# JGI-Bioinformatics/Kmernator

Measured on AMD Instinct MI355X. Metric: total k-mers/sec at k=31, 150 bp reads (spectrum build, inputs resident in HBM), higher is better.
Workload: dtype u64

## Files before the change

kmernator_amd/csrc/kmr_api.hip:

```cpp
#include <hip/hip_runtime.h>
#include <dlfcn.h>
#include <unistd.h>
#include <rccl/rccl.h>

#include <algorithm>
#include <atomic>
#include <cmath>
#include <cstdio>
#include <cstdlib>
#include <cstring>
#include <cctype>
#include <memory>
#include <mutex>
#include <string>
#include <type_traits>
#include <vector>

#include "kmr_host.hpp"
#include "kmr_kernels.hpp"
#include "kmr_partition.hpp"
#include "kmr_superkmer.hpp"
#include "kmr_buckets.hpp"
#include "kmr_synth.hpp"
#define KMR_INSTANCES_EXTERN
// ... 29 lines not shown
		if (i < 33 + (int)minQ) P[raw] = 0.0;
		else if (i < 103) P[raw] = 1.0 - pow(10.0, ((33 - i) / 10.0));
		else P[raw] = 1.0;
	}
}

}

namespace {

template <int W, class F> auto with_win(uint32_t win, F &&f) {
	if (W > 1 && win == 32) return f(int_c<(W > 1 ? 32 : 16)>());
	return win == 16 ? f(int_c<16>()) : (win == 8 ? f(int_c<8>()) : f(int_c<4>()));
}

size_t slot_bytes(kmr_handle *h) { return with_w(h, [](auto W) { return sizeof(Slot<W()>); }); }

ReadsView reads_view(const void *bases, const void *quals, const void *offsets, uint64_t n_reads, const void *discarded = nullptr, uint64_t stream_base = 0, uint64_t first_read_idx = 0) {
	ReadsView rv{};
	rv.bases = (const uint8_t *)bases; rv.quals = (const uint8_t *)quals; rv.offsets = (const uint64_t *)offsets; rv.discarded = (const uint8_t *)discarded;
	rv.n_reads = n_reads; rv.stream_base = stream_base; rv.first_read_idx = first_read_idx;
	return rv;
}
ReadsView reads_slice(const ReadsView &all, uint64_t r, uint64_t m) {
	ReadsView rv = all;
	rv.offsets = all.offsets + r; rv.n_reads = m; rv.discarded = all.discarded ? all.discarded + r : nullptr; rv.first_read_idx = all.first_read_idx + r;
	return rv;
}
FinalizeParams finalize_params(kmr_handle *h, uint32_t min_depth) {
	FinalizeParams f{};
	f.kb = h->hkb; f.ext_min_q = h->cfg.ext_min_quality; f.min_depth = min_depth; f.has_singletons = h->cfg.separate_singletons ? 1 : 0; f.nb_weak = h->nb_weak; f.nb_sing = h->nb_sing;
	return f;
}

DevParams dev_params(kmr_handle *h) {
	DevParams p;
	p.k = h->k; p.kb = h->hkb; p.min_weight = h->cfg.min_weight; p.fastq_start = h->cfg.fastq_start_char; p.ext_min_q = h->cfg.ext_min_quality;
	p.qzero = h->cfg.fastq_start_char + std::max<uint32_t>(1u, h->cfg.min_quality_score);
	p.subsample = h->cfg.kmer_subsample; p.rank = h->cfg.rank; p.world = h->cfg.world_size; p.num_parts = h->cfg.num_parts; p.part_idx = h->cfg.part_idx;
	p.count_sender_bad = h->sender_launch ? 1u : 0u;
	p.P = h->dP.get<double>(); p.stats = h->dstats.get<DevStats>(); p.err = h->derr.get<uint32_t>();
	p.sub_wstart = p.sub_wkeys = p.sub_sstart = p.sub_skeys = nullptr; p.sub_wvals = nullptr; p.sub_sweight = nullptr; p.sub_wnb = p.sub_snb = 0; p.sub_vw = 0;
	if (h->subtract) {
		const kmr_handle *o = h->subtract;
		if (o->weak.present && o->weak.n) { p.sub_wstart = o->weak.start.get<uint64_t>(); p.sub_wkeys = o->weak.keys.get<uint64_t>(); p.sub_wvals = o->weak.vals.get<uint32_t>(); p.sub_wnb = o->weak.nb; p.sub_vw = o->ext ? 15 : 3; }
		if (o->sing.present && o->sing.n) { p.sub_sstart = o->sing.start.get<uint64_t>(); p.sub_skeys = o->sing.keys.get<uint64_t>(); p.sub_sweight = o->sing.sweight.get<uint8_t>(); p.sub_snb = o->sing.nb; }
	}
	return p;
}


template <int W> Table<W> table_of(kmr_handle *h) { Table<W> t; t.slots = h->slots.get<Slot<W>>(); t.ext = h->extslots.get<ExtSlot>(); t.log2cap = h->log2cap; return t; }

template <int W> int clear_table(kmr_handle *h, void *slots, ExtSlot *ext, uint32_t log2cap) {
	hipLaunchKernelGGL(table_clear_kernel<W>, dim3(grid_for(1ull << log2cap)), dim3(256), 0, h->stream, (Slot<W> *)slots, ext, 1ull << log2cap);
	HIPCHK(h, hipGetLastError());
	return 0;
}
int clear_table_any(kmr_handle *h, void *slots, ExtSlot *ext, uint32_t log2cap) { return with_w(h, [&](auto W) { return clear_table<W()>(h, slots, ext, log2cap); }); }

int alloc_table(kmr_handle *h, uint32_t log2cap, DevBuf &slots, DevBuf &ext) {
	DevBuf s, x;
	HIPCHK(h, s.alloc(slot_bytes(h) << log2cap));
	if (h->ext) HIPCHK(h, x.alloc(sizeof(ExtSlot) << log2cap));
	const int rc = clear_table_any(h, s.get(), x.get<ExtSlot>(), log2cap);
	if (rc) return rc;
	slots = std::move(s); ext = std::move(x);
	return 0;
}

int sync_state(kmr_handle *h) {
	HIPCHK(h, hipStreamSynchronize(h->stream));
	for (int which = 0; which < KMR_TIME_GROUPS; which++) {
		for (auto &pr : h->pending_events[which]) {
			float ms = 0; hipEventElapsedTime(&ms, pr.first, pr.second);
			h->ms[which] += ms; h->launches[which]++;
			hipEventDestroy(pr.first); hipEventDestroy(pr.second);
		}
		h->pending_events[which].clear();
	}
	uint32_t e = 0; DevStats s;
	HIPCHK(h, hipMemcpy(&e, h->derr.get<uint32_t>(), sizeof(e), hipMemcpyDeviceToHost));
	HIPCHK(h, hipMemcpy(&s, h->dstats.get<DevStats>(), sizeof(s), hipMemcpyDeviceToHost));
#ifdef KMR_DEBUG_HOOKS
	if (h->superkmer_mode) { if (dbg()) fprintf(stderr, "sk_extract windows: %llu general, %llu fast\n", s.claimed, s.inserted); s.claimed = 0; s.inserted = 0; }
#endif
	h->stats.raw_kmers = s.raw + s.inserted + s.sender_bad; h->stats.raw_good_kmers = s.good + s.inserted; h->stats.discarded = s.raw - s.good + s.sender_bad;
	h->occupied = s.claimed; h->pending_kmers = 0; h->subtracted = s.subtracted;
	if (e & ERR_READ_TOO_LONG) return fail(h, KMR_ERR_UNSUPPORTED, "a read is longer than the per-wavefront LDS tile (" + std::to_string(TILE_SPAN) + " bases)");
	if (e & ERR_TABLE_FULL) return fail(h, KMR_ERR_CAPACITY, "device k-mer table is full; raise kmr_config.max_table_entries / estimated_raw_kmers");
	if (e & ERR_SEGMENT_OVERFLOW) return fail(h, KMR_ERR_CAPACITY, "an owner segment overflowed seg_capacity");
	if (e & ERR_POOL_FULL) return fail(h, KMR_ERR_CAPACITY, "record pool overflow (internal sizing error)");
	if (e & ERR_ENTRIES_FULL) return fail(h, KMR_ERR_CAPACITY, "entry buffer overflow (internal sizing error)");
	return 0;
}

template <int W, bool EXT> int grow_table_t(kmr_handle *h, uint32_t newlog) {
	DevBuf ns, ne;
	int rc = alloc_table(h, newlog, ns, ne);
	if (rc) return rc;
	Table<W> src = table_of<W>(h), dst; dst.slots = ns.get<Slot<W>>(); dst.ext = ne.get<ExtSlot>(); dst.log2cap = newlog;
	hipLaunchKernelGGL((rehash_kernel<W, EXT>), dim3(grid_for(1ull << h->log2cap)), dim3(256), 0, h->stream, src, dst, h->hkb, h->derr.get<uint32_t>());
	HIPCHK(h, hipGetLastError());
	HIPCHK(h, hipStreamSynchronize(h->stream));
	h->slots = std::move(ns); h->extslots = std::move(ne); h->log2cap = newlog;
	return 0;
}
int grow_table(kmr_handle *h, uint32_t newlog) { return with_w_ext(h, [&](auto W, auto EXT) { return grow_table_t<W(), EXT()>(h, newlog); }); }

int ensure_capacity(kmr_handle *h, uint64_t incoming) {
	const uint64_t cap = 1ull << h->log2cap;
	if ((double)(h->occupied + h->pending_kmers + incoming) <= 0.85 * (double)cap) { h->pending_kmers += incoming; return 0; }
	int rc = sync_state(h);
	if (rc) return rc;
	if ((double)(h->occupied + incoming) > 0.85 * (double)cap) {
		uint32_t nl = h->log2cap;
		while ((double)(h->occupied + incoming) > 0.6 * (double)(1ull << nl)) nl++;
		rc = grow_table(h, nl);
		if (rc) return rc;
	}
	h->pending_kmers = incoming;
	return 0;
}

const size_t EXTRACT_SMEM = (size_t)WAVES_PER_BLOCK * 2 * TILE_BUF;

int prepare_units(kmr_handle *h, ReadsView &rv, uint32_t span = (uint32_t)TILE_SPAN) {
	rv.u_start = rv.u_end = rv.u_read = nullptr; rv.n_units = 0;
	const uint64_t n = rv.n_reads;
	if (n == 0) return 0;
	int rc = h->umax.reserve(h, "umax", 4); if (rc) return rc;
	HIPCHK(h, hipMemsetAsync(h->umax.get<unsigned int>(), 0, 4, h->stream));
	rc = h->ucnt.reserve(h, "ucnt", 4 * (n + 1)); if (rc) return rc;
	hipLaunchKernelGGL(unit_count_kernel, dim3(grid_for(n)), dim3(256), 0, h->stream, rv.offsets, n, h->k, span, h->ucnt.get<uint32_t>(), h->umax.get<unsigned int>());
	HIPCHK(h, hipGetLastError());
	unsigned int mx = 0;
	HIPCHK(h, hipMemcpyAsync(&mx, h->umax.get<unsigned int>(), 4, hipMemcpyDeviceToHost, h->stream));
	HIPCHK(h, hipStreamSynchronize(h->stream));
	if (mx <= span) return 0;
	rc = h->ufirst.reserve(h, "ufirst", 8 * (n + 1)); if (rc) return rc;
	rc = exclusive_scan(h, h->ucnt.get<uint32_t>(), n, h->ufirst.get<uint64_t>()); if (rc) return rc;
	uint64_t U = 0;
	HIPCHK(h, hipMemcpy(&U, h->ufirst.get<uint64_t>() + n, 8, hipMemcpyDeviceToHost));
	if (h->u_read.cap() < 8 * U) {
		h->u_start.reset(); h->u_end.reset(); h->u_read.reset();
		HIPCHK(h, h->u_start.alloc(8 * U)); HIPCHK(h, h->u_end.alloc(8 * U)); HIPCHK(h, h->u_read.alloc(8 * U));
	}
	hipLaunchKernelGGL(unit_fill_kernel, dim3(grid_for(n)), dim3(256), 0, h->stream, rv.offsets, n, h->k, span, h->ufirst.get<uint64_t>(), h->u_start.get<uint64_t>(), h->u_end.get<uint64_t>(), h->u_read.get<uint64_t>());
	HIPCHK(h, hipGetLastError());
	rv.u_start = h->u_start.get<uint64_t>(); rv.u_end = h->u_end.get<uint64_t>(); rv.u_read = h->u_read.get<uint64_t>(); rv.n_units = U;
	return 0;
}

template <int W, bool EXT, class Op> int launch_extract(kmr_handle *h, const ReadsView &rv, const Op &op, uint64_t max_blocks = 0) {
	const DevParams dp = dev_params(h);
	const bool sub = Op::NEEDS_WEIGHT && (dp.sub_wnb | dp.sub_snb) != 0;
	auto kern = sub ? extract_kernel<W, EXT, Op, true> : extract_kernel<W, EXT, Op, false>;
	HIPCHK(h, hipFuncSetAttribute((const void *)kern, hipFuncAttributeMaxDynamicSharedMemorySize, (int)EXTRACT_SMEM));
	if (dbg()) { int nb = 0; hipOccupancyMaxActiveBlocksPerMultiprocessor(&nb, (const void *)kern, WAVES_PER_BLOCK * 64, EXTRACT_SMEM); fprintf(stderr, "extract: %d blocks of %d waves per CU (dynamic LDS %zu)\n", nb, WAVES_PER_BLOCK, EXTRACT_SMEM);
		for (size_t tr : {(size_t)79872, (size_t)65536, (size_t)52000, (size_t)38000}) { hipOccupancyMaxActiveBlocksPerMultiprocessor(&nb, (const void *)kern, WAVES_PER_BLOCK * 64, tr); fprintf(stderr, "   with %zu bytes: %d blocks\n", tr, nb); } }
	const uint64_t tiles = ((rv.u_start ? rv.n_units : rv.n_reads) + 63) / 64;
	uint64_t blocks = (tiles + WAVES_PER_BLOCK - 1) / WAVES_PER_BLOCK;
	if (blocks == 0) return 0;
	if (max_blocks && blocks > max_blocks) blocks = max_blocks;
	if (blocks > 0x7fffffffull) return fail(h, KMR_ERR_INVALID_ARG, "too many reads in one batch");
	hipLaunchKernelGGL(kern, dim3((unsigned)blocks), dim3(WAVES_PER_BLOCK * 64), EXTRACT_SMEM, h->stream, rv, dp, op);
	HIPCHK(h, hipGetLastError());
	return 0;
}

template <int W, bool EXT> int add_reads_dev_t(kmr_handle *h, const ReadsView &rvAll, uint64_t total_bases) {
	const uint64_t n = rvAll.n_reads;
	const uint64_t avg = n ? std::max<uint64_t>(1, total_bases / n) : 1;
	uint64_t chunk = std::max<uint64_t>(64, ((1ull << 27) / avg) & ~63ull);
	std::vector<uint64_t> off2(2);
	for (uint64_t r = 0; r < n; r += chunk) {
		const uint64_t m = std::min(chunk, n - r);
		HIPCHK(h, hipMemcpyAsync(&off2[0], rvAll.offsets + r, 8, hipMemcpyDeviceToHost, h->stream));
		HIPCHK(h, hipMemcpyAsync(&off2[1], rvAll.offsets + r + m, 8, hipMemcpyDeviceToHost, h->stream));
		HIPCHK(h, hipStreamSynchronize(h->stream));
		const uint64_t bases = off2[1] - off2[0];
		int rc = ensure_capacity(h, bases);
		if (rc) return rc;
		ReadsView rv = reads_slice(rvAll, r, m);
		rc = prepare_units(h, rv); if (rc) return rc;
		InsertOp<W, EXT> op; op.table = table_of<W>(h);
		TimeSpan t(h, 0);
		rc = launch_extract<W, EXT>(h, rv, op);
		t.end();
		if (rc) return rc;
	}
	return 0;
}

int add_reads_dev_any(kmr_handle *h, const ReadsView &rv, uint64_t total_bases) { return with_w_ext(h, [&](auto W, auto EXT) { return add_reads_dev_t<W(), EXT()>(h, rv, total_bases); }); }

}
namespace kmr_host {
int exclusive_scan_queue(kmr_handle *h, const uint32_t *in, uint64_t n, uint64_t *out ) {
	const uint64_t nblocks = (n + SCAN_ITEMS - 1) / SCAN_ITEMS;
	const size_t eb = sizeof(unsigned long long);
	int rc = h->scan_sums.reserve(h, "scan_sums", eb * (nblocks + 1), eb * std::max<uint64_t>(nblocks + 1, 4096)); if (rc) return rc;
	unsigned long long *sums = h->scan_sums.get<unsigned long long>(), *total = sums + nblocks;
	hipLaunchKernelGGL(scan_block_sums_kernel, dim3((unsigned)nblocks), dim3(256), 0, h->stream, in, n, sums);
	hipLaunchKernelGGL(scan_sums_kernel, dim3(1), dim3(256), 0, h->stream, sums, nblocks, total);
	hipLaunchKernelGGL(scan_apply_kernel, dim3((unsigned)nblocks), dim3(256), 0, h->stream, in, n, sums, out);
	HIPCHK(h, hipGetLastError());
	return 0;
}
int exclusive_scan(kmr_handle *h, const uint32_t *in, uint64_t n, uint64_t *out ) {
	const int rc = exclusive_scan_queue(h, in, n, out); if (rc) return rc;
	HIPCHK(h, hipStreamSynchronize(h->stream));
	return 0;
}
}
namespace {

int arena_alloc(kmr_handle *h, void **out, size_t bytes) {
	const size_t need = (bytes + 255) & ~(size_t)255;
	if (h->arena && h->arena_used + need <= h->arena.cap()) { *out = h->arena.get<uint8_t>() + h->arena_used; h->arena_used += need; h->arena_want += need; return 0; }
	h->arena_want += need;
	DevBuf b;
// ... 374 lines not shown
	const int mb = max_part_bits(h);
	int T = 0; while (T < 2 * mb && (est >> T) > TARGET_LIST_RECORDS) T++;
	h->bits1 = std::max(0, std::min(mb, T + 2 - mb));
}

template <int W, bool EXT> int extract_by_owner_t(kmr_handle *h, const ReadsView &rvAll, uint64_t total_bases, void *dev_records, uint64_t seg_capacity, void *dev_seg_counts, uint32_t *dev_pos = nullptr) {
	const uint64_t n = rvAll.n_reads;
	const uint64_t avg = n ? std::max<uint64_t>(1, total_bases / n) : 1;
	const uint64_t chunk = std::max<uint64_t>(64, (SUB_BATCH_BASES / avg) & ~63ull);
	for (uint64_t r = 0; r < n; r += chunk) {
		const uint64_t m = std::min(chunk, n - r);
		ReadsView rv = reads_slice(rvAll, r, m);
		int rc = prepare_units(h, rv); if (rc) return rc;
		const uint64_t nu = rv.u_start ? rv.n_units : m;
		rc = h->kcap.reserve(h, "kcap", 4 * std::max<uint64_t>(nu + 1, 16)); if (rc) return rc;
		rc = h->koff.reserve(h, "koff", 8 * std::max<uint64_t>(nu + 1, 16)); if (rc) return rc;
		hipLaunchKernelGGL(kmer_capacity_kernel, dim3(grid_for(nu)), dim3(256), 0, h->stream, rv, h->k, h->kcap.get<uint32_t>());
		HIPCHK(h, hipGetLastError());
		rc = exclusive_scan(h, h->kcap.get<uint32_t>(), nu, h->koff.get<uint64_t>()); if (rc) return rc;
		uint64_t total_cap = 0;
		HIPCHK(h, hipMemcpy(&total_cap, h->koff.get<uint64_t>() + nu, 8, hipMemcpyDeviceToHost));
		const uint64_t tiles = (nu + 63) / 64;
		rc = h->linear.reserve(h, "linear", sizeof(typename PoolRec<W, EXT>::type) * std::max<uint64_t>(total_cap, 16)); if (rc) return rc;
		rc = h->tile_count.reserve(h, "tile_count", 4 * std::max<uint64_t>(tiles, 16)); if (rc) return rc;
		LinearOp<W, EXT, false> op; op.records = (typename PoolRec<W, EXT>::type *)h->linear.get(); op.koff = h->koff.get<uint64_t>(); op.tile_count = h->tile_count.get<uint32_t>(); op.first_read_idx = rv.first_read_idx;
		h->sender_launch = dev_pos == nullptr;
		rc = launch_extract<W, EXT>(h, rv, op);
		h->sender_launch = false;
		if (rc) return rc;
		rc = zero_work_counter(h); if (rc) return rc;
		const int grid = (int)std::min<uint64_t>((uint64_t)num_cus(h) * 8, tiles);
		OwnerFn of; of.m = 0; of.off = of.win = of.list_bits = 0;
		if (h->superkmer_mode && h->sk_exchange) { of.m = h->sk_m; of.off = h->sk_off; of.win = h->sk_win; of.list_bits = h->sk_bits; }
		if (dev_pos)
			hipLaunchKernelGGL((owner_scatter_kernel<W, EXT, true>), dim3(grid), dim3(OWNER_THREADS), 0, h->stream, (const typename PoolRec<W, EXT>::type *)h->linear.get(), h->koff.get<uint64_t>(), h->tile_count.get<uint32_t>(), tiles, h->hkb,
			                   h->cfg.world_size, (uint32_t *)dev_records, seg_capacity, (unsigned long long *)dev_seg_counts, h->work_counter.get<unsigned int>(), h->derr.get<uint32_t>(), dev_pos, of);
		else
			hipLaunchKernelGGL((owner_scatter_kernel<W, EXT>), dim3(grid), dim3(OWNER_THREADS), 0, h->stream, (const typename PoolRec<W, EXT>::type *)h->linear.get(), h->koff.get<uint64_t>(), h->tile_count.get<uint32_t>(), tiles, h->hkb,
			                   h->cfg.world_size, (uint32_t *)dev_records, seg_capacity, (unsigned long long *)dev_seg_counts, h->work_counter.get<unsigned int>(), h->derr.get<uint32_t>(), (uint32_t *)nullptr, of);
		HIPCHK(h, hipGetLastError());
	}
	return 0;
}

template <int W, bool EXT> int add_reads_partition_t(kmr_handle *h, const ReadsView &rvAll, uint64_t total_bases) {
	const uint64_t n = rvAll.n_reads;
	if (!h->l1.head) choose_bits1(h, total_bases);
	const uint64_t avg = n ? std::max<uint64_t>(1, total_bases / n) : 1;
	const uint64_t sub_bases = h->tune.sub_batch_bases ? h->tune.sub_batch_bases : SUB_BATCH_BASES;
	const uint64_t chunk = std::max<uint64_t>(64, (sub_bases / avg) & ~63ull);
	for (uint64_t r = 0; r < n; r += chunk) {
		const uint64_t m = std::min(chunk, n - r);
		ReadsView rv = reads_slice(rvAll, r, m);
		int rc = prepare_units(h, rv); if (rc) return rc;
		const uint64_t nu = rv.u_start ? rv.n_units : m;
		rc = h->kcap.reserve(h, "kcap", 4 * std::max<uint64_t>(nu + 1, 16)); if (rc) return rc;
		rc = h->koff.reserve(h, "koff", 8 * std::max<uint64_t>(nu + 1, 16)); if (rc) return rc;
		hipLaunchKernelGGL(kmer_capacity_kernel, dim3(grid_for(nu)), dim3(256), 0, h->stream, rv, h->k, h->kcap.get<uint32_t>());
		HIPCHK(h, hipGetLastError());
		rc = exclusive_scan(h, h->kcap.get<uint32_t>(), nu, h->koff.get<uint64_t>()); if (rc) return rc;
		uint64_t total_cap = 0;
		HIPCHK(h, hipMemcpy(&total_cap, h->koff.get<uint64_t>() + nu, 8, hipMemcpyDeviceToHost));
		const uint64_t tiles = (nu + 63) / 64;
		rc = h->linear.reserve(h, "linear", rec_bytes(h) * std::max<uint64_t>(total_cap, 16)); if (rc) return rc;
		rc = h->tile_count.reserve(h, "tile_count", 4 * std::max<uint64_t>(tiles, 16)); if (rc) return rc;
		LinearOp<W, EXT> op; op.records = (typename PoolRec<W, EXT>::type *)h->linear.get(); op.koff = h->koff.get<uint64_t>(); op.tile_count = h->tile_count.get<uint32_t>(); op.first_read_idx = rv.first_read_idx;
		TimeSpan tb(h, KMR_TIME_BUILD), te(h, KMR_TIME_EXTRACT);
		rc = launch_extract<W, EXT>(h, rv, op);
		te.end();
#ifdef KMR_DEBUG_HOOKS
		if (!rc && getenv("KMR_DEBUG_SAME_TILE")) {
			const uint64_t distinct = std::max<uint64_t>(1, strtoull(getenv("KMR_DEBUG_SAME_TILE"), nullptr, 10));
			hipLaunchKernelGGL(same_tile_kernel, dim3(grid_for(tiles)), dim3(256), 0, h->stream, h->koff.get<uint64_t>(), tiles, distinct, total_cap / std::max<uint64_t>(tiles, 1));
		}
#endif
		if (!rc) rc = partition_level1<W, EXT>(h, h->linear.get(), h->koff.get<uint64_t>(), h->tile_count.get<uint32_t>(), tiles, 64, 0, 0, total_cap);
		tb.end();
		if (rc) return rc;
	}
	return 0;
}
int add_reads_partition(kmr_handle *h, const ReadsView &rv, uint64_t total_bases) { return with_w_ext(h, [&](auto W, auto EXT) { return add_reads_partition_t<W(), EXT()>(h, rv, total_bases); }); }

int build_csr(kmr_handle *h, HostPool &p, uint64_t nl, uint32_t first, uint64_t **list_start, uint64_t **list_chunks, uint32_t *n_chunks_out) {
	unsigned int used = 0;
	HIPCHK(h, hipStreamSynchronize(h->stream));
	HIPCHK(h, hipMemcpy(&used, p.head.get<unsigned int>(), 4, hipMemcpyDeviceToHost));
	if (used > p.cap) used = p.cap;
	used = used > first ? used - first : 0;
	uint32_t *cnt;
	{ int arc = arena_get(h, &cnt, nl); if (arc) return arc; arc = arena_get(h, list_start, nl + 1); if (arc) return arc;
	  arc = arena_get(h, list_chunks, std::max<unsigned>(used, 1)); if (arc) return arc; }
	HIPCHK(h, hipMemsetAsync(cnt, 0, 4 * nl, h->stream));
	const unsigned csr_grid = (unsigned)(((uint64_t)used + CSR_THREADS * CSR_ITEMS - 1) / (CSR_THREADS * CSR_ITEMS));
	if (used) hipLaunchKernelGGL(chunk_hist_kernel, dim3(csr_grid), dim3(CSR_THREADS), 0, h->stream, p.chunk_list.get<uint32_t>() + first, used, cnt, (uint32_t)nl);
	int rc = exclusive_scan(h, cnt, nl, *list_start); if (rc) return rc;
	HIPCHK(h, hipMemsetAsync(cnt, 0, 4 * nl, h->stream));
	if (used) hipLaunchKernelGGL(chunk_scatter_kernel, dim3(csr_grid), dim3(CSR_THREADS), 0, h->stream, p.chunk_list.get<uint32_t>() + first, p.chunk_count.get<uint32_t>() + first, used, first, *list_start, cnt, *list_chunks, (uint32_t)nl);
	HIPCHK(h, hipGetLastError());
	*n_chunks_out = used;
	if (dbg()) {
		unsigned long long hv[2] = {0, 0};
		DevBuf db; HIPCHK(h, db.alloc(16)); HIPCHK(h, hipMemset(db.get(), 0, 16));
		unsigned long long *d = db.get<unsigned long long>();
		if (used) hipLaunchKernelGGL(pool_records_kernel, dim3(grid_for(used)), dim3(256), 0, h->stream, p.chunk_list.get<uint32_t>(), p.chunk_count.get<uint32_t>(), used, d, d + 1);
		HIPCHK(h, hipStreamSynchronize(h->stream));
		HIPCHK(h, hipMemcpy(hv, d, 16, hipMemcpyDeviceToHost));
		fprintf(stderr, "build_csr: lists %llu chunks %u valid %llu records %llu (expected %llu)\n", (unsigned long long)nl, used, hv[1], hv[0], (unsigned long long)h->stats.raw_good_kmers);
		unsigned long long vv[3] = {0, 0, 0};
		int bits = 0; while ((1ull << bits) < nl) bits++;
		DevBuf vb; HIPCHK(h, vb.alloc(24)); HIPCHK(h, hipMemset(vb.get(), 0, 24));
		unsigned long long *v = vb.get<unsigned long long>();
		PoolView pvw = pool_view(h, p);
		with_w_ext(h, [&](auto W, auto EXT) { hipLaunchKernelGGL((verify_lists_kernel<W(), EXT()>), dim3(4096), dim3(256), 0, h->stream, pvw, *list_start, *list_chunks, nl, bits, h->hkb, part_rot(h), v, v + 1, v + 2); });
		HIPCHK(h, hipStreamSynchronize(h->stream));
		HIPCHK(h, hipMemcpy(vv, v, 24, hipMemcpyDeviceToHost));
		fprintf(stderr, "verify_lists: records via CSR %llu misfiled %llu zero-weight %llu\n", vv[0], vv[1], vv[2]);
	}
	return 0;
}

int finish_maps_from_entries(kmr_handle *h, uint32_t *wc, uint32_t *sc, uint64_t wslots, uint64_t sslots, uint64_t wn, uint64_t sn, bool keepSing, bool weak_uncounted = false, bool fixed_bins = false);
CountOut count_out(kmr_handle *h, bool packed, unsigned long long *cursors, uint32_t *wc, uint32_t *sc, FinalizeCounters *fc);

template <int W, bool EXT, int LOG2S, bool NARROW = false> int launch_count(kmr_handle *h, int grid, const uint64_t *ls, const uint64_t *lc, uint64_t nl, const CountOut &out, const FinalizeParams &f, int list_filter) {
	auto kern = count_kernel<W, EXT, LOG2S, NARROW>;
	const size_t smem = count_smem_bytes<W, EXT, LOG2S, NARROW>();
	HIPCHK(h, hipFuncSetAttribute((const void *)kern, hipFuncAttributeMaxDynamicSharedMemorySize, (int)smem));
	hipLaunchKernelGGL(kern, dim3(grid), dim3(COUNT_THREADS), smem, h->stream, pool_view(h, h->l1), ls, lc, nl, out, f, h->work_counter.get<unsigned int>(), list_filter);
	return 0;
}


struct CountPass {
	FinalizeParams f{}; bool keepSing = false, ext = false;
	bool packed = false;
	uint64_t wcap = 0, scap = 0, wmax = 0, smax = 0;
	uint32_t *wc = nullptr, *sc = nullptr; FinalizeCounters *fc = nullptr; unsigned long long *cursors = nullptr;
	FinalizeCounters c{}; unsigned long long cur[2] = {0, 0};
};

uint64_t entry_slack(uint64_t slabs) { return slabs * 8192 + 16; }
uint64_t sk_entry_slack(kmr_handle *h) { return entry_slack((uint64_t)num_cus(h) * 4); }

int count_entry_buffers(kmr_handle *h, CountPass &p, uint64_t G, uint64_t slack, uint64_t wfirst, uint64_t sfirst, bool adopted) {
	const uint64_t wbound = p.f.has_singletons ? G / 2 : G, sbound = p.keepSing ? G : 0;
	p.wmax = adopted ? (1ull << 40) : wbound + wbound / 8 + slack; p.smax = p.keepSing ? (adopted ? (1ull << 40) : sbound + sbound / 8 + slack) : 16;
	p.wcap = std::min<uint64_t>(p.wmax, wfirst + slack); p.scap = p.keepSing ? std::min<uint64_t>(p.smax, sfirst + slack) : 16;
	if (h->tune.entry_share >= 0) {
		const uint64_t n = (uint64_t)((double)G * h->tune.entry_share) + 16384;
		p.wcap = std::min<uint64_t>(p.wmax, n); if (p.keepSing) p.scap = std::min<uint64_t>(p.smax, n);
		if (p.packed) h->ue.reset(); else { h->uw_keys.reset(); h->uw_vals.reset(); }
		h->us_keys.reset(); h->us_b8.reset(); h->us_pkt.reset();
	}
	p.wcap = std::max(p.wcap, p.packed ? packed_entries(h, h->ue) : key_entries(h, h->uw_keys)); p.scap = std::max(p.scap, key_entries(h, h->us_keys));
	int rc = arena_get(h, &p.wc, h->nb_weak); if (rc) return rc; rc = arena_get(h, &p.sc, h->nb_sing); if (rc) return rc;
	rc = arena_get(h, &p.fc, 1); if (rc) return rc; rc = arena_get(h, &p.cursors, 2); if (rc) return rc;
	return 0;
}
int ensure_weak_apart(kmr_handle *h, uint64_t n, uint32_t vw) {
	if (key_entries(h, h->uw_keys) >= n && h->uw_vals) return 0;
	h->uw_keys.reset(); h->uw_vals.reset();
	HIPCHK(h, h->uw_keys.alloc(8ull * h->W * n)); HIPCHK(h, h->uw_vals.alloc(4ull * vw * n));
	return 0;
}
int ensure_entry_buffers(kmr_handle *h, const CountPass &p) {
	if (!p.packed) { const int rc = ensure_weak_apart(h, p.wcap, p.ext ? 15 : 3); if (rc) return rc; }
	else if (packed_entries(h, h->ue) < p.wcap) { h->ue.reset(); HIPCHK(h, h->ue.alloc(8ull * (h->W + 1) * p.wcap)); }
	if (key_entries(h, h->us_keys) < p.scap || !h->us_b8 || (p.ext && !h->us_pkt)) {
		h->us_keys.reset(); h->us_b8.reset(); h->us_pkt.reset();
		HIPCHK(h, h->us_keys.alloc(8ull * h->W * p.scap)); HIPCHK(h, h->us_b8.alloc(p.scap)); if (p.ext) HIPCHK(h, h->us_pkt.alloc(4 * p.scap));
	}
	return 0;
}
int count_clear(kmr_handle *h, const CountPass &p) {
	HIPCHK(h, hipMemsetAsync(p.wc, 0, 4 * h->nb_weak, h->stream)); HIPCHK(h, hipMemsetAsync(p.sc, 0, 4 * h->nb_sing, h->stream));
	HIPCHK(h, hipMemsetAsync(p.fc, 0, sizeof(FinalizeCounters), h->stream)); HIPCHK(h, hipMemsetAsync(p.cursors, 0, 16, h->stream));
	return 0;
}
int count_read_back(kmr_handle *h, CountPass &p, uint32_t &err) {
	HIPCHK(h, hipMemcpyAsync(&p.c, p.fc, sizeof(p.c), hipMemcpyDeviceToHost, h->stream)); HIPCHK(h, hipMemcpyAsync(p.cur, p.cursors, 16, hipMemcpyDeviceToHost, h->stream));
// ... 303 lines not shown
	}
	if (!weakDone) { rc = exclusive_scan(h, wc, wm.nb, wm.start.get<uint64_t>()); if (rc) return rc; }
	if (keepSing) { rc = h->bb_overflow ? exclusive_scan_queue(h, sc, sm.nb, sm.start.get<uint64_t>()) : exclusive_scan(h, sc, sm.nb, sm.start.get<uint64_t>()); if (rc) return rc; }
	else HIPCHK(h, hipMemsetAsync(sm.start.get<uint64_t>(), 0, 8 * (sm.nb + 1), h->stream));
	if (!weakDone) {
		rc = wm.keys.reserve(h, "weak map keys", std::max<uint64_t>(8ull * W * wm.n, 8)); if (rc) return rc;
		rc = wm.vals.reserve(h, "weak map vals", std::max<uint64_t>(4ull * vw * wm.n, 8)); if (rc) return rc;
	}
	rc = sm.keys.reserve(h, "singleton map keys", std::max<uint64_t>(8ull * W * sm.n, 8)); if (rc) return rc;
	rc = sm.sweight.reserve(h, "singleton map sweight", std::max<uint64_t>(sm.n, 8)); if (rc) return rc;
	if (h->ext) { rc = sm.spkt.reserve(h, "singleton map spkt", std::max<uint64_t>(4 * sm.n, 8)); if (rc) return rc; }
	HIPCHK(h, hipMemsetAsync(wc, 0, 4 * wm.nb, h->stream)); HIPCHK(h, hipMemsetAsync(sc, 0, 4 * sm.nb, h->stream));
	if (weakDone) {  }
	else if (wm.n && vw > 4) hipLaunchKernelGGL((entry_scatter_kernel<W, true>), dim3(grid_for(wslots)), dim3(256), 0, h->stream, (const uint64_t *)h->uw_keys.get(), (const uint32_t *)h->uw_vals.get(),
	                            (const uint8_t *)nullptr, (const uint32_t *)nullptr, wslots, vw, h->hkb, wm.nb, wm.start.get<uint64_t>(), wc, wm.keys.get<uint64_t>(), wm.vals.get<uint32_t>(), (uint8_t *)nullptr, (uint32_t *)nullptr);
	else if (wm.n) {
		unsigned long long *cur64 = nullptr;
		if (h->superkmer_mode && arena_get(h, &cur64, wm.nb) == 0) HIPCHK(h, hipMemcpyAsync(cur64, wm.start.get<uint64_t>(), 8 * wm.nb, hipMemcpyDeviceToDevice, h->stream));
		else cur64 = nullptr;
		hipLaunchKernelGGL(entry_scatter_kernel<W>, dim3(grid_for(wslots)), dim3(256), 0, h->stream, (const uint64_t *)h->uw_keys.get(), (const uint32_t *)h->uw_vals.get(),
		                            (const uint8_t *)nullptr, (const uint32_t *)nullptr, wslots, vw, h->hkb, wm.nb, wm.start.get<uint64_t>(), wc, wm.keys.get<uint64_t>(), wm.vals.get<uint32_t>(), (uint8_t *)nullptr, (uint32_t *)nullptr, cur64, 6);
	}
	if (sm.n) hipLaunchKernelGGL(entry_scatter_kernel<W>, dim3(grid_for(sslots)), dim3(256), 0, h->stream, (const uint64_t *)h->us_keys.get(), (const uint32_t *)nullptr,
	                            (const uint8_t *)h->us_b8.get(), (const uint32_t *)h->us_pkt.get(), sslots, 0u, h->hkb, sm.nb, sm.start.get<uint64_t>(), sc, sm.keys.get<uint64_t>(), (uint32_t *)nullptr, sm.sweight.get<uint8_t>(), h->ext ? sm.spkt.get<uint32_t>() : (uint32_t *)nullptr);
	HIPCHK(h, hipGetLastError());
	SortView<W> sv; sv.keys = wm.keys.get<uint64_t>(); sv.vals = wm.vals.get<uint32_t>(); sv.b8 = nullptr; sv.pkt = nullptr; sv.vw = vw;
	if (weakDone) {  }
	else if (h->ext) hipLaunchKernelGGL((sort_buckets_kernel<W, 15>), dim3(grid_for(wm.nb, 4, 1 << 20)), dim3(256), 0, h->stream, sv, wm.start.get<uint64_t>(), wm.nb);
	else hipLaunchKernelGGL((sort_buckets_kernel<W, 3>), dim3(grid_for(wm.nb, 4, 1 << 20)), dim3(256), 0, h->stream, sv, wm.start.get<uint64_t>(), wm.nb);
	if (sm.n) {
		SortView<W> ss; ss.keys = sm.keys.get<uint64_t>(); ss.vals = nullptr; ss.b8 = sm.sweight.get<uint8_t>(); ss.pkt = h->ext ? sm.spkt.get<uint32_t>() : nullptr; ss.vw = 0;
		hipLaunchKernelGGL((sort_buckets_kernel<W, 0>), dim3(grid_for(sm.nb, 4, 1 << 20)), dim3(256), 0, h->stream, ss, sm.start.get<uint64_t>(), sm.nb);
	}
	HIPCHK(h, hipGetLastError());
	if (!h->bb_overflow) HIPCHK(h, hipStreamSynchronize(h->stream));
	return 0;
}
int finish_maps_from_entries(kmr_handle *h, uint32_t *wc, uint32_t *sc, uint64_t wslots, uint64_t sslots, uint64_t wn, uint64_t sn, bool keepSing, bool weak_uncounted, bool fixed_bins) {
	return with_w(h, [&](auto W) { return finish_maps_t<W()>(h, wc, sc, wslots, sslots, wn, sn, keepSing, weak_uncounted, fixed_bins); });
}
int finalize_partition(kmr_handle *h, uint32_t min_depth) { return with_w_ext(h, [&](auto W, auto EXT) { return finalize_partition_t<W(), EXT()>(h, min_depth); }); }
template <int W, bool EXT> int insert_records_partition_t(kmr_handle *h, const void *recs, uint64_t n) {
	if (!h->l1.head) choose_bits1(h, n);
	TimeSpan t(h, 0);
	return partition_level1<W, EXT>(h, recs, nullptr, nullptr, (n + 8191) / 8192, 0, 8192, n, n, &h->dstats.get<DevStats>()->inserted,
	                             2 * W + (h->ext ? 2 : 1), h->stream_base);
}
int insert_records_partition(kmr_handle *h, const void *recs, uint64_t n) { return with_w_ext(h, [&](auto W, auto EXT) { return insert_records_partition_t<W(), EXT()>(h, recs, n); }); }
bool sk_geometry(uint32_t k, uint32_t m_wish, uint32_t &win, uint32_t &m, uint32_t &off, uint32_t win_max = 16) {
	for (uint32_t w : {32u, 16u, 8u, 4u}) {
		if (w > win_max) continue;
		if (w == 32u && (k < 45u || (m_wish && m_wish < 14u))) continue;
		if (k < w + 9) continue;
		uint32_t mm = std::min<uint32_t>(m_wish ? m_wish : 16u, k - w + 1);
		if (mm > 16) mm = 16;
		if (((k - mm + 1 - w) & 1u) != 0) mm--;
		if (mm < 10 && !m_wish) continue;
		if (mm < 4) continue;
		win = w; m = mm; off = (k - mm + 1 - w) / 2;
		return true;
	}
	return false;
}
const uint64_t SK_EXTRACT_WAVES_PER_CU = std::max(2 * SK_WAVES, SKL_MIN_BLOCKS * SKL_WAVES);
template <typename... P, typename... A> int launch_sk_tiles(kmr_handle *h, void (*kern)(ReadsView, P...), const char *name, int w, int win, int waves, int per_cu, size_t smem, const ReadsView &rv, const SkParams &sp, A... args) {
	HIPCHK(h, hipFuncSetAttribute((const void *)kern, hipFuncAttributeMaxDynamicSharedMemorySize, (int)smem));
	const uint64_t tiles = ((rv.u_start ? rv.n_units : rv.n_reads) + 63) / 64;
	uint64_t blocks = (tiles + waves - 1) / waves;
	if (blocks == 0) return 0;
	blocks = std::min<uint64_t>(blocks, (uint64_t)num_cus(h) * per_cu);
	if (dbg()) { int nb = 0; hipOccupancyMaxActiveBlocksPerMultiprocessor(&nb, (const void *)kern, waves * 64, smem); fprintf(stderr, "%s<W=%d,WIN=%d>: %d blocks of %d waves per CU (LDS %zu), grid %llu, m=%u off=%u bits=%u\n", name, w, win, nb, waves, smem, (unsigned long long)blocks, sp.m, sp.off, sp.list_bits); }
	hipLaunchKernelGGL(kern, dim3((unsigned)blocks), dim3(waves * 64), smem, h->stream, rv, args...);
	HIPCHK(h, hipGetLastError());
	return 0;
}
template <int W, int WIN, bool FILT, bool EXT = false> int launch_sk_extract(kmr_handle *h, const ReadsView &rv, const SkParams &sp, const DevParams *override_params = nullptr) {
	return launch_sk_tiles(h, sk_extract_kernel<W, WIN, FILT, EXT>, "sk_extract", W, WIN, SK_WAVES, 2, SK_EXTRACT_SMEM, rv, sp, override_params ? *override_params : dev_params(h), sp, pool_view(h, h->l1));
}
uint32_t sk_dbg_flags(const char *name);
bool sp_debug_extract(kmr_handle *h) { (void)h; return sk_dbg_flags("KMR_SK_EXTRACT_DBG") != 0; }
template <int W, int WIN, bool PACKED = false> int launch_sk_extract_lean(kmr_handle *h, const ReadsView &rv, const SkParams &sp, float wK, const DevParams *override_params = nullptr, const SkPacked *packed = nullptr) {
	return launch_sk_tiles(h, sk_extract_lean_kernel<W, WIN, PACKED>, "sk_extract_lean", W, WIN, SKL_WAVES, SKL_MIN_BLOCKS, SKL_EXTRACT_SMEM, rv, sp, override_params ? *override_params : dev_params(h), sp, pool_view(h, h->l1), wK, PACKED ? *packed : SkPacked{});
}
int sk_uniform_weight(kmr_handle *h, const ReadsView &rv, bool &lean, float &wK) {
	lean = false; wK = 1.0f;
	if (h->tune.no_lean_extract) return 0;
	if (!rv.quals && h->uniform_q_hint < 0) { lean = true; return 0; }
	if (h->qual_mixed || rv.n_reads == 0) return 0;
	if (h->uniform_q_hint >= 0) {
		const unsigned int q0 = (unsigned int)h->uniform_q_hint;
		if (q0 == 127) { lean = true; wK = 1.0f; return 0; }
		if (!(h->hP[q0] > 0.0)) return 0;
		lean = true; wK = (float)h->hPk[q0];
		return 0;
	}
	{ int rc = h->qrange.reserve(h, "qrange", 8); if (rc) return rc; }
	const unsigned int init[2] = {255u, 0u};
	HIPCHK(h, hipMemcpyAsync(h->qrange.get<unsigned int>(), init, 8, hipMemcpyHostToDevice, h->stream));
	hipLaunchKernelGGL(sk_qual_range_kernel, dim3(num_cus(h) * 8), dim3(256), 0, h->stream, rv.quals, rv.offsets, rv.n_reads, h->qrange.get<unsigned int>());
	HIPCHK(h, hipGetLastError());
	unsigned int got[2] = {0, 0};
	HIPCHK(h, hipMemcpyAsync(got, h->qrange.get<unsigned int>(), 8, hipMemcpyDeviceToHost, h->stream));
	HIPCHK(h, hipStreamSynchronize(h->stream));
	if (got[0] != got[1]) { h->qual_mixed = got[0] < got[1]; return 0; }
	const unsigned int q0 = got[0];
	if (q0 == 127) { lean = true; wK = 1.0f; return 0; }
	if (!(h->hP[q0] > 0.0)) return 0;
	lean = true; wK = (float)h->hPk[q0];
	return 0;
}
uint32_t sk_dbg_flags(const char *name) {
#ifdef KMR_DEBUG_HOOKS
	const char *e = getenv(name); return e ? (uint32_t)atoi(e) : 0u;
#else
	(void)name; return 0u;
#endif
}
SkParams sk_params(kmr_handle *h) { SkParams sp; sp.dbg = sk_dbg_flags("KMR_SK_EXTRACT_DBG"); sp.keep_all_owners = h->sk_exchange ? 1u : 0u; sp.track = nullptr; sp.m = h->sk_m; sp.off = h->sk_off; sp.list_bits = h->sk_bits; sp.state = h->sk_state.get<unsigned long long>(); sp.Pk = h->dPk.get<double>(); sp.Rp = h->dPk.get<double>() + 256; sp.fast_div = h->sk_fast_div ? 1u : 0u; return sp; }
template <int W> int add_reads_superkmer_t(kmr_handle *h, const ReadsView &rvAll, uint64_t total_bases) {
	const uint64_t n = rvAll.n_reads;
	const DevParams dp = dev_params(h);
	const bool filt = dp.subsample > 1 || dp.num_parts > 1 || (dp.sub_wnb | dp.sub_snb) != 0 || (dp.world > 1 && !h->sk_exchange);
	bool lean = false; float wK = 1.0f;
	if (!filt && !h->ext && !sp_debug_extract(h)) { int rcq = sk_uniform_weight(h, rvAll, lean, wK); if (rcq) return rcq; }
	if (h->packed_direct && (!lean || h->cfg.size_tracker)) return fail(h, KMR_ERR_STATE, "internal: a packed batch handed to an extraction that wants text");
	if (rvAll.n_reads) {
		uint32_t wb; memcpy(&wb, &wK, 4);
		if (!lean) h->sk_uni_mixed = true;
		else if (h->sk_uni_w == SK_UNI_NONE) h->sk_uni_w = wb;
		else if (h->sk_uni_w != wb) h->sk_uni_mixed = true;
	}
	if (!h->sk_state) {
		const uint64_t est = h->cfg.estimated_raw_kmers ? h->cfg.estimated_raw_kmers : std::max<uint64_t>(total_bases, h->call_bases_hint) * std::max<uint32_t>(1, h->cfg.world_size);
		const uint64_t per_list = h->ext ? (W > 1 ? 400 : 600) : ((h->tune.target_list == 2048 && W > 1) ? 700 : h->tune.target_list * 3 / 4);
		uint32_t bits = 6; while (bits < 24 && (est >> bits) > per_list) bits++;
		h->sk_fine_shift = 0;
		if (h->sk_exchange && h->cfg.world_size > 1 && !h->tune.no_coarse_lists) {
			uint32_t sh = 0; while ((1u << sh) < h->cfg.world_size) sh++;
			if (bits >= 6 + sh) { h->sk_fine_shift = sh; bits -= sh; }
		}
		h->sk_bits = bits;
		if (h->cfg.world_size <= 1 && !h->sk_exchange && h->tune.target_list == 2048 && !h->tune.pow2_lists) {
			const uint64_t aim = h->tune.list_aim ? h->tune.list_aim : (W == 1 ? (h->ext ? 800 : (lean ? 1450 : 1700)) : per_list * 19 / 20);
			const uint64_t nlists = (est / aim + 63) & ~63ull;
			if (nlists > 64 && (nlists < (1ull << bits) || h->tune.list_aim) && nlists < (1ull << 31)) h->sk_bits = (uint32_t)nlists;
		}
		const uint64_t nl0 = sk_list_count(h->sk_bits);
		HIPCHK(h, h->sk_state.alloc(8 * nl0));
		hipLaunchKernelGGL(sk_state_init_kernel, dim3(grid_for(nl0)), dim3(256), 0, h->stream, h->sk_state.get<unsigned long long>(), nl0);
		HIPCHK(h, hipGetLastError());
	}
	const uint64_t avg = n ? std::max<uint64_t>(1, total_bases / n) : 1;
	const uint64_t sub_bases = h->tune.sub_batch_bases ? h->tune.sub_batch_bases : (1ull << 31);
	const uint64_t chunk = std::max<uint64_t>(64, (sub_bases / avg) & ~63ull);
	if (h->cfg.size_tracker && n) {
		h->trk_n = 0;
		{ int rc = h->trk.reserve(h, "trk", n * sizeof(SkTrackRec)); if (rc) return rc; }
		HIPCHK(h, hipMemsetAsync(h->trk.get<SkTrackRec>(), 0, n * sizeof(SkTrackRec), h->stream));
	}
	for (uint64_t r = 0; r < n; r += chunk) {
		const uint64_t m = std::min(chunk, n - r);
		ReadsView rv = reads_slice(rvAll, r, m);
		int rc = prepare_units(h, rv, h->packed_direct ? SK_PACKED_SPAN : (uint32_t)TILE_SPAN); if (rc) return rc;
		const uint64_t bases = m * avg + avg;
		if (!h->l1.base && r == 0 && h->cfg.world_size <= 1 && !h->sk_exchange && (h->cfg.estimated_raw_kmers || h->call_bases_hint > total_bases)) {
			const double job_bases = h->cfg.estimated_raw_kmers ? (double)h->cfg.estimated_raw_kmers * (double)avg / (double)(avg > h->k ? avg - h->k + 1 : 1) : (double)h->call_bases_hint;
			const double rest = job_bases - (double)total_bases;
			size_t fr = 0, tot = 0;
			if (rest > 0 && hipMemGetInfo(&fr, &tot) == hipSuccess) {
				const uint64_t want = (uint64_t)(rest * (h->ext ? 2.0 : 1.0) * (lean ? 0.3 : 0.65) / SK_CHUNK_G);
				h->l1.presize = std::min<uint64_t>(want, (uint64_t)(fr / 4) / ((size_t)CH * rec_bytes(h)));
			}
		}
		rc = pool_reserve(h, h->l1, (h->ext ? 2 : 1) * bases / SK_CHUNK_G + ((h->l1.base && !h->sk_exchange) ? 0 : sk_list_count(h->sk_bits)) + (uint64_t)num_cus(h) * SK_EXTRACT_WAVES_PER_CU * 130 + 64, true); if (rc) return rc;
		TimeSpan tb(h, KMR_TIME_BUILD), te(h, KMR_TIME_EXTRACT);
		SkParams sp = sk_params(h);
		if (h->cfg.size_tracker) sp.track = h->trk.get<SkTrackRec>() + r;
		if (h->packed_direct) {
			SkPacked pkd = *h->packed_direct; pkd.off += r; if (pkd.mk_off) pkd.mk_off += r;
			rc = with_win<W>(h->sk_win, [&](auto WIN) { return launch_sk_extract_lean<W, WIN(), true>(h, rv, sp, wK, nullptr, &pkd); });
		} else rc = with_win<W>(h->sk_win, [&](auto WIN) {
			if (h->ext) return filt ? launch_sk_extract<W, WIN(), true, true>(h, rv, sp) : launch_sk_extract<W, WIN(), false, true>(h, rv, sp);
			if (filt) return launch_sk_extract<W, WIN(), true>(h, rv, sp);
			return lean ? launch_sk_extract_lean<W, WIN()>(h, rv, sp, wK) : launch_sk_extract<W, WIN(), false>(h, rv, sp);
		});
		te.end(); tb.end();
		if (rc) return rc;
	}
	if (h->cfg.size_tracker && n) {
		std::vector<SkTrackRec> recs(n);
		HIPCHK(h, hipMemcpyAsync(recs.data(), h->trk.get<SkTrackRec>(), n * sizeof(SkTrackRec), hipMemcpyDeviceToHost, h->stream));
		HIPCHK(h, hipStreamSynchronize(h->stream));
		std::vector<SkBoundary> bd; std::vector<uint64_t> good_before;
		const bool walkable = (dp.sub_wnb | dp.sub_snb) == 0;
		for (uint64_t r = 0; r < n; r++) {
			while ((uint64_t)h->trk_next <= h->trk_raw + recs[r].raw) {
				SkBoundary b; b.read = r; b.t = (uint32_t)((uint64_t)h->trk_next - h->trk_raw); b.good = 0; b.ordinal = 0;
				if (!walkable) { b.t = recs[r].raw; b.good = recs[r].good; b.ordinal = recs[r].end_ordinal; }
				bd.push_back(b); good_before.push_back(h->trk_good);
				h->trk_snap_raw.push_back(walkable ? (uint64_t)h->trk_next : h->trk_raw + recs[r].raw);
				h->trk_next = (long)((double)h->trk_next * 1.05);
				if (!walkable) break;
			}
			if (!walkable) while ((uint64_t)h->trk_next <= h->trk_raw + recs[r].raw) h->trk_next = (long)((double)h->trk_next * 1.05);
			h->trk_raw += recs[r].raw; h->trk_good += recs[r].good;
		}
		if (h->trk_bounds.size() + bd.size() > SK_TRACK_MAX) return fail(h, KMR_ERR_UNSUPPORTED, "size tracker: more than 512 elements");
		if (!bd.empty() && walkable) {
			DevBuf dbdb; HIPCHK(h, dbdb.alloc(bd.size() * sizeof(SkBoundary)));
			SkBoundary *dbd = dbdb.get<SkBoundary>();
			hipError_t e = hipMemcpyAsync(dbd, bd.data(), bd.size() * sizeof(SkBoundary), hipMemcpyHostToDevice, h->stream);
			if (e == hipSuccess) {
				ReadsView rv = rvAll; rv.u_start = rv.u_end = rv.u_read = nullptr; rv.n_units = 0;
				hipLaunchKernelGGL(sk_track_boundary_kernel<W>, dim3((unsigned)((bd.size() + 63) / 64)), dim3(64), 0, h->stream, rv, dp, dbd, (uint32_t)bd.size());
				e = hipGetLastError();
			}
			if (e == hipSuccess) e = hipMemcpyAsync(bd.data(), dbd, bd.size() * sizeof(SkBoundary), hipMemcpyDeviceToHost, h->stream);
			if (e == hipSuccess) e = hipStreamSynchronize(h->stream);
			if (e != hipSuccess) return fail(h, KMR_ERR_HIP, std::string("size tracker boundaries: ") + hipGetErrorString(e));
		}
		for (size_t i = 0; i < bd.size(); i++) { h->trk_bounds.push_back(bd[i].ordinal); h->trk_snap_good.push_back(good_before[i] + bd[i].good); }
	}
	return 0;
}
int add_reads_superkmer(kmr_handle *h, const ReadsView &rv, uint64_t total_bases) { return with_w(h, [&](auto W) { return add_reads_superkmer_t<W()>(h, rv, total_bases); }); }
static const uint64_t SAT_BATCH_BYTES = 1ull << 30;
static const uint64_t SAT_BATCH_KEYS = (1ull << 23) - 1;
static const uint64_t SAT_PAIR_BYTES = 24;
template <int W> int saturated_fix_t(kmr_handle *h, const uint64_t *ls, const uint64_t *lc, uint64_t nl, unsigned long long n_clamped, unsigned long long n_sightings, uint32_t has_singletons) {
	DevMap &wm = h->weak;
	h->last_saturated_keys = 0; h->last_saturated_batches = 0;
	if (!n_clamped || !wm.n) return 0;
	uint32_t list_bits = 0; while ((1ull << list_bits) < nl) list_bits++;
	if ((1ull << list_bits) != nl) list_bits = (uint32_t)nl;
	auto no_mem = [&](const char *what, size_t bytes) { return fail(h, KMR_ERR_OOM, std::string("saturated-key pass (weights of k-mers seen 256 times or more): no device memory for ") + what + " (" + std::to_string(bytes) + " bytes)"); };
	auto dalloc = [](DevBuf &b, size_t bytes) { return b.alloc(std::max<size_t>(bytes, 256)); };
	DevBuf bfound, bentry, blist;
	if (dalloc(bfound, 8) != hipSuccess) return no_mem("a counter", 8);
	unsigned long long *dfound = bfound.get<unsigned long long>(); uint64_t *d_entry = nullptr; uint32_t *d_list = nullptr;
	uint64_t cap = std::min<uint64_t>(wm.n, 4 * n_clamped + 1024);
	unsigned long long found = 0;
	for (;;) {
		if (dalloc(bentry, 8 * cap) != hipSuccess || dalloc(blist, 4 * cap) != hipSuccess) return no_mem("the key list", 12 * cap);
		d_entry = bentry.get<uint64_t>(); d_list = blist.get<uint32_t>();
		HIPCHK(h, hipMemsetAsync(dfound, 0, 8, h->stream));
		hipLaunchKernelGGL(sat_find_kernel<W>, dim3(grid_for(wm.n)), dim3(256), 0, h->stream, (const uint64_t *)wm.keys.get<uint64_t>(), (const uint32_t *)wm.vals.get<uint32_t>(), wm.n, h->sk_m, h->sk_off, h->sk_win, list_bits, dfound, cap, d_entry, d_list, h->ext ? 15u : 3u);
		HIPCHK(h, hipGetLastError());
		HIPCHK(h, hipMemcpyAsync(&found, dfound, 8, hipMemcpyDeviceToHost, h->stream)); HIPCHK(h, hipStreamSynchronize(h->stream));
		if (found <= cap) break;
		cap = found;
	}
	if (!found) return 0;
	std::vector<uint64_t> entry(found); std::vector<uint32_t> lst(found);
	HIPCHK(h, hipMemcpy(entry.data(), d_entry, 8 * found, hipMemcpyDeviceToHost)); HIPCHK(h, hipMemcpy(lst.data(), d_list, 4 * found, hipMemcpyDeviceToHost));
	std::vector<uint64_t> order(found);
	for (uint64_t i = 0; i < found; i++) order[i] = i;
	std::sort(order.begin(), order.end(), [&](uint64_t a, uint64_t b) { return lst[a] != lst[b] ? lst[a] < lst[b] : entry[a] < entry[b]; });
	std::vector<uint64_t> sentry(found); std::vector<uint32_t> dl; std::vector<uint64_t> le0, le1;
	for (uint64_t i = 0; i < found; i++) {
		sentry[i] = entry[order[i]];
		const uint32_t l = lst[order[i]];
		if (dl.empty() || dl.back() != l) { dl.push_back(l); le0.push_back(i); le1.push_back(i + 1); } else le1.back() = i + 1;
	}
	std::vector<uint64_t>().swap(entry); std::vector<uint32_t>().swap(lst); std::vector<uint64_t>().swap(order);
	HIPCHK(h, hipMemcpy(d_entry, sentry.data(), 8 * found, hipMemcpyHostToDevice));
	HIPCHK(h, hipMemcpy(d_list, dl.data(), 4 * dl.size(), hipMemcpyHostToDevice));
	std::vector<uint64_t> c0(dl.size()), c1(dl.size());
	{
		DevBuf bc0, bc1;
		if (dalloc(bc0, 8 * dl.size()) != hipSuccess || dalloc(bc1, 8 * dl.size()) != hipSuccess) return no_mem("the chunk ranges", 16 * dl.size());
// ... 189 lines not shown
	if (hn > cap) return fail(h, KMR_ERR_CAPACITY, "long-list work items (internal sizing error)");
	p.n_items = hn;
	if (p.n_items) {
		p.lgMain.long_threshold = LONG_CHUNKS;
		p.lgItems.item_c0 = ic0; p.lgItems.item_c1 = ic1; p.lgItems.n_items = p.n_items; p.lgItems.merge_used = dn;
	}
	return 0;
}
CountOut count_out(kmr_handle *h, bool packed, unsigned long long *cursors, uint32_t *wc, uint32_t *sc, FinalizeCounters *fc) {
	CountOut out{};
	if (packed) { out.wentries = h->ue.get<uint64_t>(); out.wcap = packed_entries(h, h->ue); }
	else { out.wkeys = h->uw_keys.get<uint64_t>(); out.wvals = h->uw_vals.get<uint32_t>(); out.wcap = key_entries(h, h->uw_keys); out.spkt = h->us_pkt.get<uint32_t>(); out.weakCount = wc; }
	out.wcursor = cursors; out.scursor = cursors + 1;
	out.skeys = h->us_keys.get<uint64_t>(); out.sweight = h->us_b8.get<uint8_t>(); out.scap = key_entries(h, h->us_keys);
	out.singCount = sc; out.fc = fc; out.err = h->derr.get<uint32_t>();
	return out;
}
template <int W> int sk_count_pass(kmr_handle *h, SkFinalize<W> &p) {
	const uint64_t nl = p.nl, n_items = p.n_items; const SkTrackView &tv = p.tv;
	uint32_t merge_log2 = 16;
	DevBuf mslots, mext;
	return count_attempts(h, p, [&]() -> int { mslots.reset(); mext.reset(); return 0; }, [&](const CountOut &out, bool repeated, uint32_t &repeat_on) -> int {
		if (repeated) merge_log2 += 3;
		int rc = 0;
		const int grid = (int)std::min<uint64_t>((uint64_t)num_cus(h) * 4, (nl / p.lgMain.list_stride + SK_LBATCH) / SK_LBATCH);
		SkCountLaunch<W> k;
		rc = sk_count_select<W>(h, p.ext, p.tracking, p.uni, k); if (rc) return rc;
		if (p.tracking) HIPCHK(h, hipMemsetAsync(tv.d_unique, 0, 8 * (tv.n + 1), h->stream));
		if (dbg()) { int nb = 0; hipOccupancyMaxActiveBlocksPerMultiprocessor(&nb, (const void *)k.kern, SKC_THREADS, k.smem); fprintf(stderr, "sk_count<W=%d>: %d blocks per CU (LDS %zu), %llu lists, %u chunks\n", W, nb, k.smem, (unsigned long long)nl, p.nch); }
		hipLaunchKernelGGL(k.kern, dim3(grid), dim3(SKC_THREADS), k.smem, h->stream, pool_view(h, h->l1), p.ls, p.lc, nl, h->k, out, p.f, h->work_counter.get<unsigned int>(), sk_dbg_flags("KMR_SK_COUNT_DBG"), tv, p.lgMain);
		HIPCHK(h, hipGetLastError());
		if (!n_items) return 0;
		SkLong<W> &lgItems = p.lgItems;
		if (mslots.alloc(sizeof(Slot<W>) << merge_log2) != hipSuccess) return fail(h, KMR_ERR_OOM, "merge table of the long lists");
		if (p.ext && mext.alloc(sizeof(ExtSlot) << merge_log2) != hipSuccess) return fail(h, KMR_ERR_OOM, "merge table of the long lists");
		hipLaunchKernelGGL(table_clear_kernel<W>, dim3(grid_for(1ull << merge_log2)), dim3(256), 0, h->stream, mslots.get<Slot<W>>(), mext.get<ExtSlot>(), 1ull << merge_log2);
		lgItems.merge.slots = mslots.get<Slot<W>>(); lgItems.merge.ext = mext.get<ExtSlot>(); lgItems.merge.log2cap = merge_log2;
		HIPCHK(h, hipMemsetAsync(lgItems.merge_used, 0, 8, h->stream));
		rc = zero_work_counter(h); if (rc) return rc;
		const int grid2 = (int)std::min<uint64_t>((uint64_t)num_cus(h) * 4, n_items);
		hipLaunchKernelGGL(k.kern, dim3(grid2), dim3(SKC_THREADS), k.smem, h->stream, pool_view(h, h->l1), p.ls, p.lc, nl, h->k, out, p.f, h->work_counter.get<unsigned int>(), sk_dbg_flags("KMR_SK_COUNT_DBG"), tv, lgItems);
		hipLaunchKernelGGL(sk_merge_emit_kernel<W>, dim3(grid_for(1ull << merge_log2)), dim3(256), 0, h->stream, lgItems.merge, out, p.f);
		if (hipGetLastError() != hipSuccess) return fail(h, KMR_ERR_HIP, "long-list launches");
		if (merge_log2 < 30) repeat_on = ERR_TABLE_FULL;
		return 0;
	});
}
template <int W> int sk_append_early(kmr_handle *h, SkFinalize<W> &p) {
	FinalizeCounters &c = p.c; const FinalizeCounters &early_c = p.early_c; unsigned long long *cur = p.cur; const uint64_t early_slots = p.early_slots;
	const size_t eb = 8ull * (W + 1);
	if (cur[0] + early_slots > packed_entries(h, h->ue)) {
		DevBuf bigger;
		HIPCHK(h, bigger.alloc(eb * (cur[0] + early_slots + 4096)));
		HIPCHK(h, hipMemcpyAsync(bigger.get(), h->ue.get(), eb * cur[0], hipMemcpyDeviceToDevice, h->stream)); HIPCHK(h, hipStreamSynchronize(h->stream));
		h->ue = std::move(bigger);
	}
	HIPCHK(h, hipMemcpyAsync((uint8_t *)h->ue.get<uint64_t>() + eb * cur[0], h->early.ue.get<uint64_t>(), eb * early_slots, hipMemcpyDeviceToDevice, h->stream));
	cur[0] += early_slots;
	c.unique += early_c.unique; c.singletons += early_c.singletons; c.weak_kept += early_c.weak_kept; c.sing_kept += early_c.sing_kept;
	c.saturated += early_c.saturated; c.sat_sightings += early_c.sat_sightings;
	h->stats.unique_kmers = c.unique; h->stats.singleton_kmers = p.f.has_singletons ? c.singletons : 0;
	return 0;
}

template <int W> int finalize_superkmer_t(kmr_handle *h, uint32_t min_depth) {
	int rc = sync_state(h);
	if (rc) return rc;
	TimeSpan whole(h, KMR_TIME_FINALIZE);
	const uint64_t G = h->stats.raw_good_kmers;
	SkFinalize<W> p;
	p.f = finalize_params(h, min_depth);
	p.keepSing = p.f.has_singletons && min_depth <= 1;
	p.ext = h->ext; p.packed = !p.ext;
	p.tracking = h->cfg.size_tracker != 0;
	if (!h->l1.head) { rc = pool_reserve(h, h->l1, 0, false); if (rc) return rc; }
	rc = arena_reset(h); if (rc) return rc;
	p.nl = h->sk_state ? sk_list_count(h->sk_bits) : 1;
	if (h->sk_state) {
		hipLaunchKernelGGL(sk_close_kernel, dim3(grid_for(p.nl)), dim3(256), 0, h->stream, h->sk_state.get<unsigned long long>(), p.nl, h->l1.chunk_count.get<uint32_t>(), h->l1.cap);
		HIPCHK(h, hipGetLastError());
	}
	p.refined = h->sk_state && h->sk_fine_shift > 0;
	if (p.refined) { rc = sk_refine_lists(h, p.nl); if (rc) return rc; }
	rc = build_csr(h, h->l1, p.nl, 0, &p.ls, &p.lc, &p.nch); if (rc) return rc;
	rc = count_entry_buffers(h, p, G, sk_entry_slack(h), G / (p.f.has_singletons ? 8 : 3), G / 3, h->sk_exchange && h->cfg.world_size > 1); if (rc) return rc;
	rc = sk_count_uniform<W>(h, p.tracking, p.uni, p.f.uni_wbits); if (rc) return rc;
	h->last_count_uniform = p.uni;
	if (p.tracking) { rc = sk_track_view(h, p.tv); if (rc) return rc; }
	p.lgMain = sk_own_lists<W>(h, p.refined);
	bool device_error = false;
	rc = sk_early_takeover<W>(h, p, min_depth, device_error); if (rc) return rc;
	if (device_error) { whole.end(); return sync_state(h); }
	rc = sk_long_items<W>(h, p); if (rc) return rc;
	rc = sk_count_pass<W>(h, p); if (rc) return rc;
	h->stats.unique_kmers = p.c.unique;
	h->stats.singleton_kmers = p.f.has_singletons ? p.c.singletons : 0;
	if (p.tracking) { rc = sk_track_elements(h, p.tv, p.f.has_singletons); if (rc) return rc; }
	if (p.early_slots) { rc = sk_append_early<W>(h, p); if (rc) return rc; }
	h->early.active = false;
	{ TimeSpan t(h, KMR_TIME_BUCKETS); rc = finish_maps_from_entries(h, p.wc, p.sc, p.cur[0], p.cur[1], p.c.weak_kept, p.c.sing_kept, p.keepSing, p.packed, h->tune.bb_fixed_bins); }
	if (rc) return rc;
	h->last_bb_fallback = false;
	if (h->bb_overflow) {
		uint32_t ovf = 0;
		HIPCHK(h, hipMemcpyAsync(&ovf, h->bb_overflow, 4, hipMemcpyDeviceToHost, h->stream)); HIPCHK(h, hipStreamSynchronize(h->stream));
		h->bb_overflow = nullptr;
		if (ovf) {
			if (dbg()) fprintf(stderr, "bucket build: a bin of the radix partition overflowed its capacity, again with measured bins\n");
			h->last_bb_fallback = true;
			rc = sk_count_pass<W>(h, p); if (rc) return rc;
			if (p.early_slots) { rc = sk_append_early<W>(h, p); if (rc) return rc; }
			{ TimeSpan t(h, KMR_TIME_BUCKETS); rc = finish_maps_from_entries(h, p.wc, p.sc, p.cur[0], p.cur[1], p.c.weak_kept, p.c.sing_kept, p.keepSing, p.packed, false); }
			if (rc) return rc;
		}
	}
	h->last_saturated_keys = 0; h->last_saturated_batches = 0;
	if (p.c.saturated) { rc = saturated_fix_t<W>(h, p.ls, p.lc, p.nl, p.c.saturated, p.c.sat_sightings, p.f.has_singletons); if (rc) return rc; }
	whole.end();
	return publish_maps(h, p.keepSing);
}
template <int W> int count_prefix_superkmer_t(kmr_handle *h, uint32_t min_depth, uint64_t hi) {
	int rc = sync_state(h); if (rc) return rc;
	FinalizeParams f = finalize_params(h, min_depth);
	const bool keepSing = f.has_singletons && min_depth <= 1;
	h->early.active = false;
	if (h->ext || h->cfg.size_tracker || keepSing || (h->sk_state && h->sk_fine_shift > 0) || !h->sk_state) return KMR_OK;
	const uint64_t nl = sk_list_count(h->sk_bits);
	if (hi > nl) hi = nl;
	if (hi == 0) return KMR_OK;
	rc = arena_reset(h); if (rc) return rc;
	hipLaunchKernelGGL(sk_close_kernel, dim3(grid_for(nl)), dim3(256), 0, h->stream, h->sk_state.get<unsigned long long>(), nl, h->l1.chunk_count.get<uint32_t>(), h->l1.cap);
	HIPCHK(h, hipGetLastError());
	uint64_t *ls = nullptr, *lc = nullptr; uint32_t nch = 0;
	rc = build_csr(h, h->l1, nl, 0, &ls, &lc, &nch); if (rc) return rc;
	const uint64_t G = h->stats.raw_good_kmers;
	uint64_t want = (uint64_t)((double)G * ((double)hi / (double)nl) / (f.has_singletons ? 6.0 : 2.5)) + sk_entry_slack(h);
	if (h->tune.early_entry_share >= 0) { want = (uint64_t)((double)G * h->tune.early_entry_share) + 16384; h->early.ue.reset(); }
	rc = h->early.ue.reserve(h, "early count ue", 8ull * (W + 1) * want); if (rc) return rc;
	rc = h->early.cursor.reserve(h, "early count cursor", 16); if (rc) return rc;
	rc = h->early.fc.reserve(h, "early count fc", sizeof(FinalizeCounters)); if (rc) return rc;
	rc = h->early.err.reserve(h, "early count error word", 4); if (rc) return rc;
	HIPCHK(h, hipMemsetAsync(h->early.cursor.get<unsigned long long>(), 0, 16, h->stream)); HIPCHK(h, hipMemsetAsync(h->early.fc.get(), 0, sizeof(FinalizeCounters), h->stream));
	HIPCHK(h, hipMemsetAsync(h->early.err.get<uint32_t>(), 0, 4, h->stream));
	bool uni = false;
	if (!h->peer_uni_mixed) { rc = sk_count_uniform<W>(h, false, uni, f.uni_wbits); if (rc) return rc; }
	const SkTrackView tv{};
	SkLong<W> lg = sk_own_lists<W>(h, false);
	lg.long_threshold = h->tune.long_list_chunks ? h->tune.long_list_chunks : 1024;
	uint32_t *sc = nullptr;
	rc = arena_get(h, &sc, h->nb_sing); if (rc) return rc;
	HIPCHK(h, hipMemsetAsync(sc, 0, 4 * h->nb_sing, h->stream));
	CountOut out{};
	out.wentries = h->early.ue.get<uint64_t>(); out.wcursor = h->early.cursor.get<unsigned long long>(); out.wcap = packed_entries(h, h->early.ue);
	out.scursor = h->early.cursor.get<unsigned long long>() + 1;
	out.singCount = sc; out.fc = (FinalizeCounters *)h->early.fc.get(); out.err = h->early.err.get<uint32_t>();
	rc = zero_work_counter(h); if (rc) return rc;
	const uint64_t n_work = hi > lg.list_first ? (hi - lg.list_first + lg.list_stride - 1) / lg.list_stride : 0;
	if (n_work) {
		const int grid = (int)std::min<uint64_t>((uint64_t)num_cus(h) * 4, (n_work + SK_LBATCH) / SK_LBATCH);
		SkCountLaunch<W> k;
		rc = sk_count_select<W>(h, false, false, uni, k); if (rc) return rc;
		TimeSpan t(h, KMR_TIME_COUNT);
		hipLaunchKernelGGL(k.kern, dim3(grid), dim3(SKC_THREADS), k.smem, h->stream, pool_view(h, h->l1), ls, lc, hi, h->k, out, f, h->work_counter.get<unsigned int>(), sk_dbg_flags("KMR_SK_COUNT_DBG"), tv, lg);
		t.end();
		HIPCHK(h, hipGetLastError());
	}
	h->early.active = true; h->early.hi = hi; h->early.min_depth = min_depth;
	return KMR_OK;
}
int count_prefix_superkmer(kmr_handle *h, uint32_t min_depth, uint64_t hi) { return with_w(h, [&](auto W) { return count_prefix_superkmer_t<W()>(h, min_depth, hi); }); }
int finalize_superkmer(kmr_handle *h, uint32_t min_depth) { return with_w(h, [&](auto W) { return finalize_superkmer_t<W()>(h, min_depth); }); }

template <class M> void release(kmr_handle *h) { static_cast<M &>(*h) = M(); }

void free_partition_state(kmr_handle *h) {
	release<BuildMem>(h);
	if (h->tb_copy_stream) { hipStreamDestroy(h->tb_copy_stream); h->tb_copy_stream = nullptr; for (int a = 0; a < 2; a++) { hipEventDestroy(h->tb_ready[a]); hipEventDestroy(h->tb_consumed[a]); h->tb_set_used[a] = false; } }
}

}

extern "C" {

uint32_t kmr_abi_version(void) { return KMR_ABI_VERSION; }

int kmr_config_init(kmr_config *c) {
	if (!c) return KMR_ERR_INVALID_ARG;
	memset(c, 0, sizeof(*c));
	c->struct_size = sizeof(*c);
	c->value_kind = KMR_VALUE_COUNT_DIR; c->min_weight = 0.10f; c->min_quality_score = 3; c->fastq_start_char = 33;
	c->ext_min_quality = 20; c->separate_singletons = 1; c->kmer_subsample = 1; c->device = -1; c->rank = 0; c->world_size = 1;
	c->estimated_depth = 20.0; c->estimated_error_rate = 0.35; c->kmers_per_bucket = 32; c->num_parts = 1; c->part_idx = 0;
	return KMR_OK;
}

const char *kmr_last_error(const kmr_handle *h) { return h ? h->err.c_str() : g_create_error.c_str(); }

int kmr_create(const kmr_config *cfg, kmr_handle **out) {
	if (!cfg || !out) return fail(nullptr, KMR_ERR_INVALID_ARG, "null argument");
	*out = nullptr;
	if (cfg->struct_size != sizeof(kmr_config)) return fail(nullptr, KMR_ERR_INVALID_ARG, "kmr_config.struct_size mismatch (ABI)");
	if (cfg->k < 1 || cfg->k > 128) return fail(nullptr, KMR_ERR_INVALID_ARG, "k must be in 1..128");
	if (cfg->world_size < 1 || cfg->rank >= cfg->world_size) return fail(nullptr, KMR_ERR_INVALID_ARG, "bad rank/world_size");
	if (cfg->value_kind > KMR_VALUE_EXT) return fail(nullptr, KMR_ERR_INVALID_ARG, "bad value_kind");
	if (cfg->hash_kind > KMR_HASH_LOOKUP8) return fail(nullptr, KMR_ERR_INVALID_ARG, "bad hash_kind");
	int ndev = 0;
	if (hipGetDeviceCount(&ndev) != hipSuccess || ndev == 0) return fail(nullptr, KMR_ERR_NO_DEVICE, "no HIP device: this library has no CPU path");
	kmr_handle *h = new kmr_handle();
	h->cfg = *cfg;
	if (h->cfg.kmer_subsample == 0) h->cfg.kmer_subsample = 1;
	if (h->cfg.num_parts == 0) h->cfg.num_parts = 1;
	h->k = cfg->k; h->kb = (cfg->k + 3) / 4; h->W = (h->kb + 7) / 8; h->ext = cfg->value_kind == KMR_VALUE_EXT;
	h->hkb = h->kb | (cfg->hash_kind << 16);
	memset(&h->stats, 0, sizeof(h->stats));
	int rc = 0;
	do {
		if (cfg->device >= 0) { if (hipSetDevice(cfg->device) != hipSuccess) { rc = fail(nullptr, KMR_ERR_NO_DEVICE, "hipSetDevice failed"); break; } }
		if (hipGetDevice(&h->device) != hipSuccess) { rc = fail(nullptr, KMR_ERR_NO_DEVICE, "hipGetDevice failed"); break; }
		if (hipStreamCreate(&h->stream) != hipSuccess) { rc = fail(nullptr, KMR_ERR_HIP, "hipStreamCreate failed"); break; }
		uint64_t w = cfg->num_buckets_weak, s = cfg->num_buckets_singleton;
		const double depth = cfg->estimated_depth > 0 ? cfg->estimated_depth : 20.0;
		const uint32_t kpb = cfg->kmers_per_bucket ? cfg->kmers_per_bucket : 32;
		const uint64_t raw = cfg->estimated_raw_kmers / (cfg->world_size > 1 ? cfg->world_size : 1);
		if (w == 0) { unsigned long est = (unsigned long)(int)(raw / depth); w = est / kpb + 1; }
		if (s == 0) { unsigned long est = cfg->separate_singletons ? (unsigned long)(raw * cfg->estimated_error_rate) : 1; s = est / kpb + 1; }
		h->nb_weak = resize_buckets(w); h->nb_sing = resize_buckets(s);
		h->has_singletons = cfg->separate_singletons != 0;
		uint64_t want = cfg->max_table_entries ? (uint64_t)(cfg->max_table_entries / 0.7) : (uint64_t)(cfg->estimated_raw_kmers * 0.45 / 0.6);
		if (cfg->world_size > 1 && !cfg->max_table_entries) want /= cfg->world_size;
		uint32_t lg = 16; while ((1ull << lg) < want && lg < 40) lg++;
		h->log2cap = lg;
		double P[256]; quality_table(P, cfg->min_quality_score, cfg->fastq_start_char);
		if (h->dP.alloc(sizeof(P)) != hipSuccess || h->dstats.alloc(sizeof(DevStats)) != hipSuccess || h->derr.alloc(4) != hipSuccess) { rc = fail(nullptr, KMR_ERR_OOM, "hipMalloc failed"); break; }
		hipMemcpy(h->dP.get<double>(), P, sizeof(P), hipMemcpyHostToDevice); hipMemset(h->dstats.get<DevStats>(), 0, sizeof(DevStats)); hipMemset(h->derr.get<uint32_t>(), 0, 4);
		if (cfg->build_mode > 3) { rc = fail(nullptr, KMR_ERR_INVALID_ARG, "bad build_mode"); break; }
		h->partition_mode = cfg->build_mode != 1;
		uint32_t wish_w = 0, wish_m = 0, wish_o = 0;
		const bool sk_auto = cfg->build_mode == 0 && cfg->world_size <= 1 && sk_geometry(h->k, 0, wish_w, wish_m, wish_o);
		h->auto_mode = cfg->build_mode == 0;
		const bool sk_ready = sk_geometry(h->k, 0, wish_w, wish_m, wish_o);
		if (cfg->build_mode == 3 || sk_auto || sk_ready) {
			if (!sk_geometry(h->k, 0, h->sk_win, h->sk_m, h->sk_off)) { rc = fail(nullptr, KMR_ERR_UNSUPPORTED, "build_mode 3 (super-k-mer lists) needs k >= 13"); break; }
			h->superkmer_mode = cfg->build_mode == 3 || sk_auto;
			double Pk[256];
			for (int cidx = 0; cidx < 256; cidx++) { double wv = 1.0; for (uint32_t jj = 0; jj < h->k; jj++) wv *= P[cidx]; Pk[cidx] = wv; }
			memcpy(h->hPk, Pk, sizeof(Pk)); memcpy(h->hP, P, sizeof(h->hP));
			if (h->dPk.alloc(2 * sizeof(Pk)) != hipSuccess) { rc = fail(nullptr, KMR_ERR_OOM, "hipMalloc failed"); break; }
			hipMemcpy(h->dPk.get<double>(), Pk, sizeof(Pk), hipMemcpyHostToDevice);
			double Rp[256]; bool fast = true;
			for (int cidx = 0; cidx < 256; cidx++) Rp[cidx] = P[cidx] != 0.0 ? 1.0 / P[cidx] : 0.0;
			for (int a = 0; a < 256 && fast; a++) for (int b = 0; b < 256; b++) {
				if (P[a] == 0.0 || P[b] == 0.0) continue;
				const double q0 = P[a] * Rp[b];
				if (std::fma(std::fma(-q0, P[b], P[a]), Rp[b], q0) != P[a] / P[b]) { fast = false; break; }
			}
			h->sk_fast_div = fast;
			hipMemcpy(h->dPk.get<double>() + 256, Rp, sizeof(Rp), hipMemcpyHostToDevice);
		}
		if (cfg->size_tracker && (!h->superkmer_mode || h->ext || cfg->world_size > 1)) { rc = fail(nullptr, KMR_ERR_UNSUPPORTED, "size_tracker: kept by the super-k-mer build (build_mode 0 / 3, direction-counting values, k >= 13) of a single partition"); break; }
		if (!h->partition_mode) {
			rc = alloc_table(h, h->log2cap, h->slots, h->extslots);
			if (rc) { g_create_error = h->err; break; }
		}
		if (hipStreamSynchronize(h->stream) != hipSuccess) { rc = fail(nullptr, KMR_ERR_HIP, std::string("table clear failed: ") + hipGetErrorString(hipGetLastError())); break; }
	} while (0);
	if (rc) { kmr_destroy(h); return rc; }
	*out = h;
	return KMR_OK;
}

static void exchange_destroy_comm(kmr_handle *h);
void kmr_destroy(kmr_handle *h) {
	if (!h) return;
	if (h->stream) hipStreamSynchronize(h->stream);
	for (int which = 0; which < KMR_TIME_GROUPS; which++) for (auto &pr : h->pending_events[which]) { hipEventDestroy(pr.first); hipEventDestroy(pr.second); }
	release<HandleMem>(h);
	free_partition_state(h);
	exchange_destroy_comm(h);
	release<ExchangeMem>(h);
	if (h->stream) hipStreamDestroy(h->stream);
	delete h;
}

int kmr_num_buckets(const kmr_handle *h, int which, uint64_t *out) {
	if (!h || !out) return KMR_ERR_INVALID_ARG;
	if (which == KMR_MAP_WEAK) *out = h->finalized && h->weak.present ? h->weak.nb : h->nb_weak;
	else if (which == KMR_MAP_SINGLETON) *out = h->finalized && h->sing.present ? h->sing.nb : h->nb_sing;
	else return KMR_ERR_UNSUPPORTED;
	return KMR_OK;
}

int kmr_reset(kmr_handle *h) {
	if (!h) return KMR_ERR_INVALID_ARG;
	hipSetDevice(h->device);
	HIPCHK(h, hipStreamSynchronize(h->stream));
	clear_map(h->weak); clear_map(h->sing);
	int rc = 0;
	if (h->partition_mode) {
		if (h->l1.head) HIPCHK(h, hipMemsetAsync(h->l1.head.get<unsigned int>(), 0, 4, h->stream));
		h->l1.used_ub = 0;
		h->inserted_records = 0;
		h->qual_mixed = false;
		h->sk_uni_w = SK_UNI_NONE; h->sk_uni_mixed = false; h->peer_uni_w = SK_UNI_NONE; h->peer_uni_mixed = false; h->peers_declare = false;
		h->xr_lo = 0; h->xr_hi = ~0ull; h->early.active = false;
		if (h->d_uni) { const uint32_t init[2] = {SK_UNI_NONE, 0u}; HIPCHK(h, hipMemcpyAsync(h->d_uni.get<uint32_t>(), init, 8, hipMemcpyHostToDevice, h->stream)); HIPCHK(h, hipStreamSynchronize(h->stream)); }
		if (h->sk_state) hipLaunchKernelGGL(sk_state_init_kernel, dim3(grid_for(sk_list_count(h->sk_bits))), dim3(256), 0, h->stream, h->sk_state.get<unsigned long long>(), sk_list_count(h->sk_bits));
		if (h->l1_state) {
			hipLaunchKernelGGL(partition_state_init_kernel, dim3(partition_blocks(h)), dim3(256), 0, h->stream, h->l1_state.get<uint8_t>(),
			                   h->l1_state.cap() / (size_t)partition_blocks(h), h->bits1, (uint32_t)partition_blocks(h));
			h->l1_state_dirty = false;
		}
	} else {
		if (!h->slots) rc = alloc_table(h, h->log2cap, h->slots, h->extslots);
		else rc = clear_table_any(h, h->slots.get(), h->extslots.get<ExtSlot>(), h->log2cap);
		if (rc) return rc;
	}
	HIPCHK(h, hipMemsetAsync(h->dstats.get<DevStats>(), 0, sizeof(DevStats), h->stream));
	HIPCHK(h, hipMemsetAsync(h->derr.get<uint32_t>(), 0, 4, h->stream));
	memset(&h->stats, 0, sizeof(h->stats));
	h->occupied = h->pending_kmers = 0; h->stream_base = 0; h->reads = 0; h->subtracted = 0; h->xc_job_bases = 0; h->xc_bytes_to_peers = 0;
	h->trk_n = 0; h->trk_elems.clear();
	h->trk_next = 128; h->trk_raw = h->trk_good = 0; h->trk_bounds.clear(); h->trk_snap_raw.clear(); h->trk_snap_good.clear();
	h->finalized = false; h->map_gen++; h->has_singletons = h->cfg.separate_singletons != 0;
	return KMR_OK;
}
int kmr_release_table(kmr_handle *h) {
	if (!h) return KMR_ERR_INVALID_ARG;
	if (!h->finalized) return fail(h, KMR_ERR_STATE, "kmr_release_table before kmr_finalize");
	hipSetDevice(h->device);
	h->slots.reset(); h->extslots.reset();
	if (h->partition_mode) free_partition_state(h);
	return KMR_OK;
}

void *kmr_stream(kmr_handle *h) { return h ? (void *)h->stream : nullptr; }

int kmr_set_stream_origin(kmr_handle *h, uint64_t ordinal) {
	if (!h) return KMR_ERR_INVALID_ARG;
	if (h->finalized) return fail(h, KMR_ERR_STATE, "kmr_set_stream_origin after kmr_finalize");
	if (ordinal > MAX_STREAM_ORDINAL) return fail(h, KMR_ERR_CAPACITY, "stream ordinals have 40 bits");
	h->stream_base = ordinal;
	return KMR_OK;
}

int kmr_tune(kmr_handle *h, const char *knob, double value) {
	if (!h || !knob) return KMR_ERR_INVALID_ARG;
	const std::string k(knob);
	if (k == "target_list_records") h->tune.target_list = value >= 1 ? (uint64_t)value : 2048;
	else if (k == "sub_batch_bases") h->tune.sub_batch_bases = value >= 1 ? (uint64_t)value : 0;
	else if (k == "recycle_chunks") h->tune.recycle = value < 0 ? -1 : (value != 0 ? 1 : 0);
	else if (k == "partition_blocks") h->tune.part_blocks = value >= 1 ? (int)value : 0;
	else if (k == "entry_share") h->tune.entry_share = value;
	else if (k == "early_entry_share") h->tune.early_entry_share = value;
	else if (k == "saturated_batch_bytes") h->tune.saturated_batch_bytes = value >= 1 ? (uint64_t)value : 0;
	else if (k == "lookup_table") h->tune.no_lut = value == 0;
	else if (k == "stream_lookups") h->tune.no_stream_lookups = value == 0;
	else if (k == "long_list_chunks") h->tune.long_list_chunks = value < 2 ? 2 : (uint64_t)value;
	else if (k == "lean_extract") h->tune.no_lean_extract = value == 0;
	else if (k == "uniform_count") h->tune.no_uniform_count = value == 0;
	else if (k == "packed_direct") h->tune.no_packed_direct = value == 0;
	else if (k == "pow2_lists") h->tune.pow2_lists = value != 0;
	else if (k == "list_aim") h->tune.list_aim = value >= 1 ? (uint64_t)value : 0;
	else if (k == "twobit_piece_bases") h->tune.twobit_piece_bases = (uint64_t)value;
	else if (k == "exchange_fail_once") h->tune.exchange_fail_once = value != 0;
	else if (k == "binned_buckets_min") h->tune.binned_min = value >= 0 ? (uint64_t)value : ~0ull;
	else if (k == "bb_fixed_bins") h->tune.bb_fixed_bins = value != 0;
	else if (k == "bb_slack_bins") h->tune.bb_slack_bins = value;
	else if (k == "bb_slack_groups") h->tune.bb_slack_groups = value;
	else if (k == "bb_reload") h->tune.bb_reload = value != 0;
	else if (k == "coarse_lists") h->tune.no_coarse_lists = value == 0;
	else if (k == "select_timing") h->tune.select_timing = value != 0;
	else if (k == "dump_timing") h->tune.dump_timing = value != 0;
	else if (k == "pairs_timing") h->tune.pairs_timing = value != 0;
	else if (k == "dedup_timing") h->tune.dedup_timing = value != 0;
	else if (k == "partition_units") h->tune.partition_units = value >= 1 && value <= 8192 ? (uint32_t)value : 0;
	else if (k == "pair_hash_bits") h->tune.pair_hash_bits = value >= 1 && value < 64 ? (uint32_t)value : 64;
	else if (k == "dump_piece_bytes") h->tune.dump_piece_bytes = value >= 1 ? (uint64_t)value : 0;
	else if (k == "narrow_tallies") h->tune.no_narrow = value == 0;
	else if (k == "keep_level1_state") h->tune.no_l1_state = value == 0;
	else if (k == "superkmer_window") {
		if (h->superkmer_mode && !h->sk_state) { uint32_t w, m, o; if (!sk_geometry(h->k, 0, w, m, o, (uint32_t)value)) return fail(h, KMR_ERR_INVALID_ARG, "no minimizer geometry under that window"); h->sk_win = w; h->sk_m = m; h->sk_off = o; }
	}
	else if (k == "superkmer_minimizer") {
		if (h->superkmer_mode && !h->sk_state) { uint32_t w, m, o; if (!sk_geometry(h->k, (uint32_t)value, w, m, o)) return fail(h, KMR_ERR_INVALID_ARG, "no minimizer geometry for that length"); h->sk_win = w; h->sk_m = m; h->sk_off = o; }
	}
	else return fail(h, KMR_ERR_INVALID_ARG, "unknown tuning knob '" + k + "'");
	return KMR_OK;
}

int kmr_build_info(kmr_handle *h, const char *what, double *value) {
	if (!h || !what || !value) return KMR_ERR_INVALID_ARG;
	const std::string k(what);
	if (k == "lists") *value = h->sk_state ? (double)sk_list_count(h->sk_bits) : 0.0;
	else if (k == "uniform_count") *value = h->last_count_uniform ? 1.0 : 0.0;
	else if (k == "chunk_pool_chunks") *value = (double)h->l1.cap;
	else if (k == "superkmer_window") *value = (double)h->sk_win;
	else if (k == "early_lists") *value = (double)h->last_early_hi;
	else if (k == "early_entries") *value = (double)h->last_early_entries;
	else if (k == "early_overflowed") *value = h->last_early_overflowed ? 1.0 : 0.0;
	else if (k == "bb_path") *value = (double)h->last_bb_path;
	else if (k == "bb_fallback") *value = h->last_bb_fallback ? 1.0 : 0.0;
	else if (k == "score_path") *value = (double)h->last_score_path;
	else if (k == "saturated_keys") *value = (double)h->last_saturated_keys;
	else if (k == "saturated_batches") *value = (double)h->last_saturated_batches;
	else if (k == "count_attempts") *value = (double)h->last_count_attempts;
	else if (k == "device_blocks_live") *value = (double)g_blocks_live.load();
	else if (k == "filter_score_ms") *value = h->last_score_ms;
	else if (k == "select_ms") *value = h->last_select_ms;
	else if (k == "select_write_ms") *value = h->last_write_ms;
	else if (k == "pairs_ms") *value = h->last_pairs_ms;
	else if (k == "pairs_parse_ms") *value = h->last_pairs_parse_ms;
	else if (k == "pairs_sort_ms") *value = h->last_pairs_sort_ms;
	else if (k == "pair_hash_collisions") *value = (double)h->last_pair_hash_collisions;
	else if (k == "dedup_ms") *value = h->last_dedup_ms;
	else if (k == "dedup_key_ms") *value = h->last_dedup_key_ms;
	else if (k == "dedup_sort_ms") *value = h->last_dedup_sort_ms;
	else if (k == "dedup_consensus_ms") *value = h->last_dedup_consensus_ms;
	else if (k == "dump_size_ms") *value = h->last_dump_size_ms;
	else if (k == "dump_write_ms") *value = h->last_dump_write_ms;
	else return fail(h, KMR_ERR_INVALID_ARG, "unknown build figure '" + k + "'");
	return KMR_OK;
}

int kmr_sync(kmr_handle *h) { if (!h) return KMR_ERR_INVALID_ARG; hipSetDevice(h->device); return sync_state(h); }

int kmr_add_reads_dev(kmr_handle *h, const void *dev_bases, const void *dev_quals, const void *dev_offsets, uint64_t n_reads,
                      uint64_t total_bases, uint64_t first_global_read_idx, const void *dev_discarded) {
	if (!h) return KMR_ERR_INVALID_ARG;
	if (h->finalized) return fail(h, KMR_ERR_STATE, "kmr_add_reads after kmr_finalize");
	if (n_reads == 0) return KMR_OK;
	if (!dev_bases || !dev_offsets) return fail(h, KMR_ERR_INVALID_ARG, "null device buffer");
	hipSetDevice(h->device);
	const ReadsView rv = reads_view(dev_bases, dev_quals, dev_offsets, n_reads, dev_discarded, h->stream_base, first_global_read_idx);
	if (h->stream_base + total_bases > MAX_STREAM_ORDINAL) return fail(h, KMR_ERR_CAPACITY, "more than 2^40 input bases on one handle");
	if (h->partition_mode && !h->superkmer_mode && !h->ext && h->stream_base + total_bases > (1ull << 32))
		return fail(h, KMR_ERR_CAPACITY, "build_mode 2 orders occurrences by a 32-bit stream ordinal: at most 2^32 input bases per handle without extension values (use build_mode 0 / 3 or 1)");
	int rc = h->superkmer_mode ? add_reads_superkmer(h, rv, total_bases) : (h->partition_mode ? add_reads_partition(h, rv, total_bases) : add_reads_dev_any(h, rv, total_bases));
	h->stream_base += total_bases; h->reads += n_reads; h->stats.reads = h->reads;
	return rc;
}

static hipError_t tb_stage_copy(kmr_handle *h, int set, int which, const void *src, size_t bytes, void **dst) {
	DevBuf &buf = h->tb_stage[set][which];
	if (buf.cap() < bytes + 128) {
		if (buf) { hipError_t e0 = hipStreamSynchronize(h->stream); if (e0 != hipSuccess) return e0; }
		hipError_t e = buf.alloc(bytes + bytes / 8 + 4096); if (e != hipSuccess) return e;
	}
	*dst = buf.get();
	return bytes ? hipMemcpyAsync(buf.get(), src, bytes, hipMemcpyHostToDevice, h->tb_copy_stream) : hipSuccess;
}
static int tb_pipeline_ready(kmr_handle *h) {
	if (h->tb_copy_stream) return 0;
	HIPCHK(h, hipStreamCreateWithFlags(&h->tb_copy_stream, hipStreamNonBlocking));
	for (int i = 0; i < 2; i++) { HIPCHK(h, hipEventCreateWithFlags(&h->tb_ready[i], hipEventDisableTiming)); HIPCHK(h, hipEventCreateWithFlags(&h->tb_consumed[i], hipEventDisableTiming)); }
	return 0;
}

#define TBCHK(call) do { hipError_t e_ = (call); if (e_ != hipSuccess) { hipStreamSynchronize(h->tb_copy_stream); hipStreamSynchronize(h->stream); h->err = std::string(#call) + ": " + hip_err_text(e_); return e_ == hipErrorOutOfMemory ? KMR_ERR_OOM : KMR_ERR_HIP; } } while (0)
}
template <class Stage, class Feed> static int tb_feed_pieces(kmr_handle *h, const uint64_t *offsets, uint64_t n_reads, Stage &&stage, Feed &&feed) {
	{ int rcp = tb_pipeline_ready(h); if (rcp) return rcp; }
	const uint64_t piece_bases = h->tune.twobit_piece_bases ? h->tune.twobit_piece_bases : (1ull << 28);
	int rc = KMR_OK; int set = 0;
	h->call_bases_hint = n_reads ? offsets[n_reads] - offsets[0] : 0;
	struct HintReset { kmr_handle *h; ~HintReset() { h->call_bases_hint = 0; } } hint_reset{h};
	for (uint64_t r0 = 0; r0 < n_reads && rc == KMR_OK; set ^= 1) {
		uint64_t r1 = r0 + 1;
		while (r1 < n_reads && offsets[r1 + 1] - offsets[r0] <= piece_bases) r1++;
		if (h->tb_set_used[set]) TBCHK(hipStreamWaitEvent(h->tb_copy_stream, h->tb_consumed[set], 0));
		{ int rcs = stage(set, r0, r1); if (rcs) return rcs; }
		TBCHK(hipEventRecord(h->tb_ready[set], h->tb_copy_stream));
		TBCHK(hipStreamWaitEvent(h->stream, h->tb_ready[set], 0));
		rc = feed(r0, r1);
		TBCHK(hipEventRecord(h->tb_consumed[set], h->stream)); h->tb_set_used[set] = true;
		r0 = r1;
	}
	hipStreamSynchronize(h->tb_copy_stream);
	if (!rc) rc = sync_state(h);
	else hipStreamSynchronize(h->stream);
	return rc;
}
extern "C" {

int kmr_add_reads(kmr_handle *h, const char *bases, const char *quals, const uint64_t *offsets, uint64_t n_reads,
                  uint64_t first_global_read_idx, const uint8_t *discarded) {
	if (!h) return KMR_ERR_INVALID_ARG;
	if (h->finalized) return fail(h, KMR_ERR_STATE, "kmr_add_reads after kmr_finalize");
	if (n_reads == 0) return KMR_OK;
// ... 878 lines not shown
```

kmernator_amd/csrc/kmr_host.hpp:

```cpp
#ifndef KMR_HOST_HPP_
#define KMR_HOST_HPP_

#include <hip/hip_runtime.h>
#include <unistd.h>

#include <algorithm>
#include <atomic>
#include <cstdio>
#include <memory>
#include <string>
#include <type_traits>
#include <utility>
#include <vector>

#include "../../include/kmernator_amd.h"

#define KMR_HIDDEN __attribute__((visibility("hidden")))

namespace kmr { struct SkPacked; }

namespace kmr_host KMR_HIDDEN {

inline std::string g_create_error;

// ... 2 lines not shown
inline hipError_t dev_malloc(void **p, size_t bytes) {
	hipError_t e = hipMalloc(p, bytes);
	if (e == hipSuccess) { if (*p) g_blocks_live++; return e; }
	if (e != hipErrorOutOfMemory) return e;
	size_t fr = 0, tot = 0;
	for (int attempt = 0; attempt < 6; attempt++) {
		(void)hipGetLastError();
		hipDeviceSynchronize();
		if (hipMemGetInfo(&fr, &tot) != hipSuccess || bytes > tot) break;
		usleep(20000u << attempt);
		e = hipMalloc(p, bytes);
		if (e == hipSuccess && *p) g_blocks_live++;
		if (e != hipErrorOutOfMemory) return e;
	}
	(void)hipGetLastError();
	hipMemGetInfo(&fr, &tot);
	snprintf(g_oom_note, sizeof(g_oom_note), " [requested %.3f GB; device has %.3f GB free of %.3f GB]", bytes / 1e9, fr / 1e9, tot / 1e9);
	*p = nullptr;
	return hipErrorOutOfMemory;
}

class DevBuf {
public:
	DevBuf() = default;
	DevBuf(DevBuf &&o) noexcept : p_(o.p_), cap_(o.cap_) { o.p_ = nullptr; o.cap_ = 0; }
	DevBuf &operator=(DevBuf &&o) noexcept { if (this != &o) { reset(); std::swap(p_, o.p_); std::swap(cap_, o.cap_); } return *this; }
	~DevBuf() { reset(); }
	void reset() { if (p_) { hipFree(p_); g_blocks_live--; } p_ = nullptr; cap_ = 0; }
	hipError_t alloc(size_t bytes) {
		reset();
		void *p = nullptr;
		const hipError_t e = dev_malloc(&p, bytes);
		if (e == hipSuccess) { p_ = p; cap_ = bytes; }
		return e;
	}
	int reserve(kmr_handle *h, const char *what, size_t need, size_t bytes = 0);
	template <class T = void> T *get() const { return (T *)p_; }
	size_t cap() const { return cap_; }
	explicit operator bool() const { return p_ != nullptr; }
private:
	void *p_ = nullptr;
	size_t cap_ = 0;
};

struct DevMap {
	uint64_t nb = 0, n = 0;
	DevBuf start;
	DevBuf keys;
	DevBuf vals;
	DevBuf sweight;
	DevBuf spkt;
	DevBuf image;
	bool present = false;
};

struct HostPool {
	DevBuf base, chunk_list, chunk_count, head;
	uint32_t cap = 0; size_t chunk_bytes = 0;
	uint64_t used_ub = 0;
	uint64_t presize = 0;
};

struct HandleMem {
	DevBuf slots, extslots;
	DevBuf dP, dstats, derr;
	DevMap weak, sing;
	DevBuf ix_start, ix_keys, ix_counts;
	DevBuf scratch_stats;
	DevBuf adopt_buf;
	DevBuf trk;
	DevBuf scan_sums;
	DevBuf score_buf;
	DevBuf lut;
	DevBuf dPk;
	DevBuf d_uni;
	DevBuf qrange;
	DevBuf sk_fine_state;
	struct Early { bool active = false; uint64_t hi = 0; uint32_t min_depth = 0; DevBuf ue, cursor, fc, err; } early;
	DevBuf dedup_tab;
	DevBuf xo_dev;
};
struct BuildMem {
	DevBuf sk_state;
	HostPool l1;
	DevBuf work_counter;
	DevBuf l1_state; bool l1_state_dirty = false;
	DevBuf arena; size_t arena_used = 0, arena_want = 0; std::vector<DevBuf> arena_overflow;
	DevBuf linear;
	DevBuf tile_count, kcap, koff;
	DevBuf ucnt, ufirst, u_start, u_end, u_read, umax;
	DevBuf tb_bases, tb_quals, tb_rel, tb_off, tb_len;
	uint64_t tb_quals_filled = 0; int tb_quals_char = -1;
	DevBuf tb_stage[2][8];
	DevBuf uw_keys, uw_vals, us_keys, us_b8, us_pkt;
	DevBuf ue, ue2;
};
struct ExchangeMem {
	DevBuf xc_small, xc_dcounts;
	DevBuf xc_send, xc_send2, xc_recv, xc_recv2;
};

}
using namespace kmr_host;

struct KMR_HIDDEN Tuning {
	uint64_t target_list = 2048;
	uint64_t sub_batch_bases = 0;
	int recycle = -1;
	int part_blocks = 0;
	double entry_share = -1.0;
	double early_entry_share = -1.0;
	uint64_t saturated_batch_bytes = 0;
	bool no_lut = false, no_narrow = false, no_l1_state = false, no_stream_lookups = false;
	uint64_t long_list_chunks = 0;
	uint64_t binned_min = 1ull << 18;
	bool bb_fixed_bins = true;
	double bb_slack_bins = 1.0, bb_slack_groups = 1.0;
	bool bb_reload = false;
	uint64_t twobit_piece_bases = 0;
	uint64_t list_aim = 0;
	bool pow2_lists = false;
	bool no_packed_direct = false;
	bool no_uniform_count = false;
	bool no_lean_extract = false;
	bool exchange_fail_once = false;
	uint64_t dump_piece_bytes = 0;
	bool dump_timing = false;
	bool select_timing = false;
	bool pairs_timing = false;
	bool dedup_timing = false;
	uint32_t partition_units = 0;
	uint32_t pair_hash_bits = 64;
	bool no_coarse_lists = true;
};

struct KMR_HIDDEN kmr_handle : HandleMem, BuildMem, ExchangeMem {
	kmr_config cfg;
	Tuning tune;
	uint32_t k = 0, kb = 0, hkb = 0, W = 0;
	bool ext = false;
	int device = 0, ncu = 0;
	hipStream_t stream = nullptr;
	std::string err;
	uint32_t log2cap = 0;
	uint64_t occupied = 0;
	uint64_t pending_kmers = 0;
	uint64_t stream_base = 0, reads = 0;
	uint64_t nb_weak = 0, nb_sing = 0;
	bool finalized = false, has_singletons = true;
	kmr_handle *subtract = nullptr;
	uint64_t subtracted = 0;
	kmr_stats stats;
	bool partition_mode = false;
	bool superkmer_mode = false;
	uint64_t ix_lists = 0, ix_gen = ~0ull;
	uint64_t trk_n = 0; std::vector<uint64_t> trk_elems;
	long trk_next = 128; uint64_t trk_raw = 0, trk_good = 0; std::vector<unsigned long long> trk_bounds; std::vector<uint64_t> trk_snap_raw, trk_snap_good;
	bool sk_fast_div = false;
	bool sender_launch = false;
	bool sk_exchange = false;
	bool auto_mode = false;
	int bits1 = 0;
	uint64_t inserted_records = 0;
	uint64_t call_bases_hint = 0;
	uint32_t lut_log2 = 0;
	uint64_t lut_gen = ~0ull, map_gen = 0;
	hipStream_t tb_copy_stream = nullptr; hipEvent_t tb_ready[2] = {nullptr, nullptr}, tb_consumed[2] = {nullptr, nullptr}; bool tb_set_used[2] = {false, false};
	const kmr::SkPacked *packed_direct = nullptr;
	int uniform_q_hint = -1;
	uint32_t sk_bits = 0, sk_m = 0, sk_off = 0, sk_win = 0;
	double hP[256], hPk[256];
	uint32_t sk_uni_w = 0xffffffffu; bool sk_uni_mixed = false; bool last_count_uniform = false;
	uint32_t peer_uni_w = 0xffffffffu; bool peer_uni_mixed = false, peers_declare = false;
	uint64_t xr_lo = 0, xr_hi = ~0ull;
	uint64_t last_early_hi = 0, last_early_entries = 0;
	int last_bb_path = 0; bool last_bb_fallback = false; uint32_t *bb_overflow = nullptr;
	int last_score_path = 0;
	bool last_early_overflowed = false;
	double last_score_ms = 0, last_select_ms = 0, last_write_ms = 0;
	double last_dump_size_ms = 0, last_dump_write_ms = 0;
	double last_pairs_ms = 0, last_pairs_parse_ms = 0, last_pairs_sort_ms = 0;
	double last_dedup_ms = 0, last_dedup_key_ms = 0, last_dedup_sort_ms = 0, last_dedup_consensus_ms = 0;
	uint64_t last_pair_hash_collisions = 0;
	uint64_t last_saturated_keys = 0, last_saturated_batches = 0;
	int last_count_attempts = 0;
	bool qual_mixed = false;
	uint32_t sk_fine_shift = 0;
	uint32_t sk_min_override = 0;
	uint64_t xo_segcap = 0; std::vector<uint64_t> xo_counts; const void *xo_batch = nullptr; uint64_t xo_first = 0;
	void *xc_comm = nullptr; kmr_transport xc_tr = {nullptr, nullptr, nullptr};
	uint64_t xc_job_bases = 0, xc_bytes_to_peers = 0;
	hipEvent_t ev0 = nullptr, ev1 = nullptr;
	double ms[KMR_TIME_GROUPS] = {0};
	uint64_t launches[KMR_TIME_GROUPS] = {0};
	std::vector<std::pair<hipEvent_t, hipEvent_t> > pending_events[KMR_TIME_GROUPS];
};

struct OnDevice { int device = 0; };

struct KMR_HIDDEN kmr_picks : OnDevice {
	DevBuf text, picked;
	uint64_t n = 0, n_picked = 0, bytes = 0;
	DevBuf read_seg;
	std::vector<uint64_t> seg_table;
	uint32_t n_rounds = 1, n_inputs = 1;
	float round_depth[33] = {};
	uint8_t round_is_remainder[33] = {};
};

struct KMR_HIDDEN kmr_pairs : OnDevice {
	DevBuf mate, read1, read2;
	uint64_t n = 0, n_pairs = 0, n_full = 0, n_seq = 0, n_conflicts = 0;
};

struct KMR_HIDDEN kmr_text : OnDevice {
	DevBuf text;
	uint64_t kept = 0, bytes = 0;
};

struct KMR_HIDDEN kmr_reads : OnDevice {
	DevBuf bases, quals;
	DevBuf offsets;
	DevBuf name_off, name_len;
	uint64_t n = 0, total = 0, filtered = 0;
	uint32_t input_base = 0;
};

struct KMR_HIDDEN kmr_dedup : OnDevice {
	DevBuf disc, group_first, group_size, names;
	kmr_reads *cons = nullptr;
	~kmr_dedup() { delete cons; }
	uint64_t n = 0, n_groups = 0, affected = 0, name_bytes = 0;
	uint64_t skipped[4] = {0, 0, 0, 0};
};

namespace kmr_host KMR_HIDDEN {

inline std::string oom_note() { std::string s(g_oom_note); g_oom_note[0] = 0; return s; }

inline std::string hip_err_text(hipError_t e) { return std::string(hipGetErrorString(e)) + (e == hipErrorOutOfMemory ? oom_note() : std::string()); }

#define HIPCHK(h, call) do { hipError_t e_ = (call); if (e_ != hipSuccess) { \
	(h)->err = std::string(#call) + ": " + hip_err_text(e_); \
	return e_ == hipErrorOutOfMemory ? KMR_ERR_OOM : KMR_ERR_HIP; } } while (0)

inline int DevBuf::reserve(kmr_handle *h, const char *what, size_t need, size_t bytes) {
	if (p_ && cap_ >= need) return 0;
	if (!bytes) bytes = need;
	hipError_t e = p_ ? hipStreamSynchronize(h->stream) : hipSuccess;
	if (e == hipSuccess) e = alloc(bytes);
	if (e == hipSuccess) return 0;
	h->err = std::string("device buffer ") + what + " (" + std::to_string(bytes) + " bytes): " + hip_err_text(e);
	return e == hipErrorOutOfMemory ? KMR_ERR_OOM : KMR_ERR_HIP;
}

inline int fail(kmr_handle *h, int code, const std::string &msg) { const std::string m = code == KMR_ERR_OOM ? msg + oom_note() : msg; if (h) h->err = m; else g_create_error = m; return code; }

template <int N> using int_c = std::integral_constant<int, N>;
template <class F> auto with_w(const kmr_handle *h, F &&f) {
	switch (h->W) { case 1: return f(int_c<1>()); case 2: return f(int_c<2>()); case 3: return f(int_c<3>()); default: return f(int_c<4>()); }
}
template <class F> auto with_w_ext(const kmr_handle *h, F &&f) {
	return with_w(h, [&](auto W) { return h->ext ? f(W, std::true_type()) : f(W, std::false_type()); });
}

inline int grid_for(uint64_t n, int block = 256, int maxBlocks = 256 * 16) {
	uint64_t g = (n + block - 1) / block;
	if (g < 1) g = 1;
	if (g > (uint64_t)maxBlocks) g = maxBlocks;
// ... 44 lines not shown
```

kmernator_amd/csrc/kmr_kernels.hpp:

```cpp
#ifndef KMR_KERNELS_HPP_
#define KMR_KERNELS_HPP_

#include <hip/hip_runtime.h>
#include <stdint.h>
#include <string.h>

#include "kmr_key.hpp"

namespace kmr {

static const uint64_t EMPTY_KEY = ~0ull;
static const uint64_t NO_FIRST = ~0ull;

static const int FIRST_ORD_SHIFT = 24;
static const uint64_t MAX_STREAM_ORDINAL = (1ull << 40) - 1;
__host__ __device__ __forceinline__ uint32_t first_weight_bits(float w) {
#if defined(__HIP_DEVICE_COMPILE__)
	const uint32_t bits = __float_as_uint(w);
#else
	uint32_t bits; memcpy(&bits, &w, 4);
#endif
	const uint32_t ex = (bits >> 23) & 0xffu;
	if (ex == 0 || ex > 127u) return ex > 127u ? (254u << 15) : 0u;
	const uint32_t prod = ((bits & 0x7fffffu) | 0x800000u) * 254u;
	const uint32_t sh = 8u + (127u - ex);
	return sh < 32u ? prod >> sh : 0u;
}
__host__ __device__ __forceinline__ unsigned long long first_pack(uint64_t ordinal, bool forward, float w) {
	return ((unsigned long long)ordinal << FIRST_ORD_SHIFT) | ((unsigned long long)(forward ? 1u : 0u) << 23) | (unsigned long long)(first_weight_bits(w) & 0x7fffffu);
}
__host__ __device__ __forceinline__ bool first_forward(unsigned long long f) { return ((f >> 23) & 1ull) != 0; }
__host__ __device__ __forceinline__ double first_weight_shift(unsigned long long f) {
	const uint32_t q8 = (uint32_t)(f >> 15) & 0xffu, r15 = (uint32_t)f & 0x7fffu;
	const double w1 = ((double)q8 + ((double)r15 + 0.5) / 32768.0) / 254.0;
	return (double)(float)((double)q8 / 254.0) - w1;
}
static const int WAVES_PER_BLOCK = 4;
#ifndef KMR_TILE_BUF
#define KMR_TILE_BUF 9856
#endif
static const int TILE_BUF = KMR_TILE_BUF;
static const int TILE_SPAN = TILE_BUF - 32;

enum { ERR_READ_TOO_LONG = 1, ERR_TABLE_FULL = 2, ERR_SEGMENT_OVERFLOW = 4 };

struct DevStats {
	unsigned long long raw, good, claimed;
	unsigned long long inserted;
	unsigned long long subtracted;
	unsigned long long sender_bad;
};

struct DevParams {
	uint32_t k, kb;
	float min_weight;
	uint32_t fastq_start, ext_min_q;
	uint32_t qzero;
	uint32_t subsample, rank, world, num_parts, part_idx;
	uint32_t count_sender_bad;
	const double *P;
	DevStats *stats;
	uint32_t *err;
	const uint64_t *sub_wstart, *sub_wkeys; const uint32_t *sub_wvals; uint64_t sub_wnb; uint32_t sub_vw;
	const uint64_t *sub_sstart, *sub_skeys; const uint8_t *sub_sweight; uint64_t sub_snb;
};

struct ReadsView {
	const uint8_t *bases;
	const uint8_t *quals;
	const uint64_t *offsets;
	const uint8_t *discarded;
	uint64_t n_reads;
	uint64_t stream_base;
	uint64_t first_read_idx;
	const uint64_t *u_start, *u_end, *u_read;
	uint64_t n_units;
};

static const uint32_t UNIT_KMERS = 9216;
#ifndef KMR_INSTANCE_TU
__global__ void unit_count_kernel(const uint64_t *offsets, uint64_t n, uint32_t k, uint32_t span, uint32_t *counts, unsigned int *maxLen) {
	unsigned int mx = 0;
	for (uint64_t r = blockIdx.x * (uint64_t)blockDim.x + threadIdx.x; r < n; r += (uint64_t)gridDim.x * blockDim.x) {
		const uint64_t L = offsets[r + 1] - offsets[r];
		mx = L > mx ? (unsigned int)(L > 0xffffffffull ? 0xffffffffu : L) : mx;
		counts[r] = L <= span ? 1u : (uint32_t)((L - k + 1 + UNIT_KMERS - 1) / UNIT_KMERS);
	}
#pragma unroll
	for (int off = 32; off > 0; off >>= 1) { unsigned int o = __shfl_xor(mx, off, 64); mx = o > mx ? o : mx; }
	if ((threadIdx.x & 63) == 0 && mx > __hip_atomic_load(maxLen, __ATOMIC_RELAXED, __HIP_MEMORY_SCOPE_AGENT)) atomicMax(maxLen, mx);
}
#endif
#ifndef KMR_INSTANCE_TU
__global__ void unit_fill_kernel(const uint64_t *offsets, uint64_t n, uint32_t k, uint32_t span, const uint64_t *ufirst,
                                 uint64_t *u_start, uint64_t *u_end, uint64_t *u_read) {
	for (uint64_t r = blockIdx.x * (uint64_t)blockDim.x + threadIdx.x; r < n; r += (uint64_t)gridDim.x * blockDim.x) {
		const uint64_t b = offsets[r], e = offsets[r + 1], L = e - b;
		const uint64_t u0 = ufirst[r], nu = ufirst[r + 1] - u0;
		if (L <= span) { u_start[u0] = b; u_end[u0] = e; u_read[u0] = r; continue; }
		for (uint64_t g = 0; g < nu; g++) {
			const uint64_t s0 = b + g * UNIT_KMERS, e0 = s0 + UNIT_KMERS + k - 1;
			u_start[u0 + g] = s0; u_end[u0 + g] = e0 < e ? e0 : e; u_read[u0 + g] = r;
		}
	}
}
#endif

template <int W> struct Slot;
template <> struct Slot<1> {
	uint64_t key;
	unsigned long long cntfwd;
	double wsum;
	unsigned long long first;
};
template <int W> struct Slot {
	uint64_t key[W];
	unsigned long long cntfwd;
	double wsum;
	unsigned long long first;
	uint32_t state;
	uint32_t pad;
};
struct ExtSlot {
	uint32_t tally[12];
	uint32_t pkt;
	uint32_t pad[3];
};

template <int W> struct Table {
	Slot<W> *slots;
	ExtSlot *ext;
	uint32_t log2cap;
};

__device__ __forceinline__ uint64_t ld_relaxed(const uint64_t *p) {
	return __hip_atomic_load(p, __ATOMIC_RELAXED, __HIP_MEMORY_SCOPE_AGENT);
}

template <int W>
__device__ __forceinline__ uint64_t table_find_or_insert(const Table<W> &t, const Key<W> &key, uint64_t hash, bool &claimed) {
	const uint64_t mask = (1ull << t.log2cap) - 1;
	uint64_t s = table_slot(hash, t.log2cap);
	claimed = false;
	uint64_t probes = 0;
	if constexpr (W == 1) {
		for (;;) {
			uint64_t cur = t.slots[s].key;
			if (cur == key.w[0]) return s;
			if (cur == EMPTY_KEY) {
				unsigned long long old = atomicCAS((unsigned long long *)&t.slots[s].key, (unsigned long long)EMPTY_KEY, (unsigned long long)key.w[0]);
				if (old == EMPTY_KEY) { claimed = true; return s; }
				if (old == key.w[0]) return s;
			}
			s = (s + 1) & mask;
			if (++probes > mask) return ~0ull;
		}
	} else {
		for (;;) {
			uint32_t st = __hip_atomic_load(&t.slots[s].state, __ATOMIC_ACQUIRE, __HIP_MEMORY_SCOPE_AGENT);
			if (st == 0) {
				uint32_t old = atomicCAS(&t.slots[s].state, 0u, 1u);
				if (old == 0) {
// ... 1180 lines not shown
```

kmernator_amd/csrc/kmr_partition.hpp:

```cpp
#ifndef KMR_PARTITION_HPP_
#define KMR_PARTITION_HPP_

#include "kmr_kernels.hpp"

namespace kmr {

#ifndef KMR_CH
#define KMR_CH 64
#endif
static const int CH = KMR_CH;
static const uint32_t NO_CHUNK = 0xffffffffu;
enum { ERR_POOL_FULL = 8, ERR_ENTRIES_FULL = 16 };

struct PoolView {
	uint8_t *base;
	uint32_t *chunk_list;
	uint32_t *chunk_count;
	unsigned int *head;
	uint32_t cap;
	uint32_t *err;
};

__host__ __device__ __forceinline__ uint64_t mix64(uint64_t x) {
	x ^= x >> 33; x *= 0xff51afd7ed558ccdull; x ^= x >> 33; x *= 0xc4ceb9fe1a85ec53ull; x ^= x >> 33;
// ... 425 lines not shown
					s_gfirst[ng] = nb;
					s_ecur = e; s_eoff = off; s_ng = ng;
				}
				lds_barrier();
				const uint32_t ng = s_ng;
				if (ng == 0) break;
				for (uint32_t g = 0; g < ng; g++) { load1(g, r, pid); scatter_batch(r, pid, 0); }
			}
			lds_barrier();
		}
		lds_barrier();
		if (gstate && !S.state_final) {
			for (int p = t; p < P; p += THREADS) { gstate[p] = cur[p]; gstate[P + p] = cnt[p]; gstate[2 * P + p] = stage_n[p]; }
			for (int i = t; i < P * G; i += THREADS) glines[i] = stage[i];
		} else {
			flush_all(0);
			if (gstate) for (int p = t; p < P; p += THREADS) { gstate[p] = NO_CHUNK; gstate[P + p] = 0; gstate[2 * P + p] = 0; }
		}
		if (S.valid_counter) { nvalid = wave_sum(nvalid); if ((t & 63) == 0 && nvalid) atomicAdd(S.valid_counter, nvalid); }
	} else {
		uint32_t cid[RPT];
		uint64_t dsc[RPT];
		auto load_desc = [&](uint64_t cb, uint64_t cb1) {
#pragma unroll
			for (int i = 0; i < RPT; i++) { const uint64_t ci = cb + (uint64_t)i * (THREADS / CH) + (t >> 6); dsc[i] = ci < cb1 ? S.list_chunks[ci] : ~0ull; }
		};
		auto load2 = [&](uint64_t cb, uint64_t cb1, auto &rr, auto &pp) {
#pragma unroll
			for (int i = 0; i < RPT; i++) {
				const uint64_t ci = cb + (uint64_t)i * (THREADS / CH) + (t >> 6);
				pp[i] = NO_CHUNK; cid[i] = NO_CHUNK;
				if (ci < cb1) {
					const uint64_t d = dsc[i];
					const uint32_t c = (uint32_t)d;
					cid[i] = c;
					if ((uint32_t)(t & 63) < (uint32_t)(d >> 32)) {
						rr[i] = ((const Rec *)(S.src.base + (size_t)c * CH * sizeof(Rec)))[t & 63];
						pp[i] = pid_of(rr[i]);
					}
				}
			}
		};
		for (;;) {
			if (t == 0) s_item = atomicAdd(work_counter, 1u);
			lds_barrier();
			const uint64_t it = s_item;
			lds_barrier();
			if (it >= S.n_items) break;
			const uint64_t cb0 = S.item_begin[it], cb1 = S.item_end[it];
			const uint32_t lid_base = S.item_list[it] << LOG2P;
			constexpr uint64_t STEP = BATCH / CH;
			load_desc(cb0, cb1);
			for (uint64_t cb = cb0; cb < cb1; cb += STEP) {
				load2(cb, cb1, r, pid);
				load_desc(cb + STEP, cb1);
				scatter_batch(r, pid, lid_base);
				if (S.recycle && (t & 63) == 0) {
#pragma unroll
					for (int i = 0; i < RPT; i++) if (cid[i] != NO_CHUNK) {
						const int pos = atomicAdd(&s_free_n, 1);
						if (pos < FREE_CAP) s_free[pos] = cid[i];
						else { atomicSub(&s_free_n, 1); out.chunk_list[cid[i]] = NO_CHUNK; out.chunk_count[cid[i]] = 0; }
					}
				}
			}
			lds_barrier();
			flush_all(lid_base);
			lds_barrier();
		}
	}
	lds_barrier();
	if (LEVEL == 2 && S.recycle)
		for (int i = t; i < s_free_n && i < FREE_CAP; i += THREADS) { out.chunk_list[s_free[i]] = NO_CHUNK; out.chunk_count[s_free[i]] = 0; }
	for (uint32_t idx = s_alloc + t; idx < s_filled; idx += THREADS) {
		const uint32_t c = s_ring[(idx / SLAB) % RING] + (idx % SLAB);
		if (c < out.cap) { out.chunk_list[c] = NO_CHUNK; out.chunk_count[c] = 0; }
	}
}

static const int CSR_LDS_LISTS = 4096;
static const int CSR_THREADS = 256, CSR_ITEMS = 16;
#ifndef KMR_INSTANCE_TU
__global__ __launch_bounds__(CSR_THREADS)
void chunk_hist_kernel(const uint32_t *chunk_list, uint32_t n_chunks, uint32_t *list_nchunks, uint32_t nl) {
	__shared__ uint32_t lh[CSR_LDS_LISTS];
	const bool priv = nl <= (uint32_t)CSR_LDS_LISTS;
	if (priv) { for (uint32_t i = threadIdx.x; i < nl; i += CSR_THREADS) lh[i] = 0; __syncthreads(); }
	const uint64_t base = (uint64_t)blockIdx.x * CSR_THREADS * CSR_ITEMS;
	for (int j = 0; j < CSR_ITEMS; j++) {
		const uint64_t c = base + (uint64_t)j * CSR_THREADS + threadIdx.x;
		if (c >= n_chunks) break;
		const uint32_t l = chunk_list[c];
		if (l == NO_CHUNK) continue;
		if (priv) atomicAdd(&lh[l], 1u); else atomicAdd(&list_nchunks[l], 1u);
	}
	if (priv) { __syncthreads(); for (uint32_t i = threadIdx.x; i < nl; i += CSR_THREADS) if (lh[i]) atomicAdd(&list_nchunks[i], lh[i]); }
}
#endif
#ifndef KMR_INSTANCE_TU
__global__ __launch_bounds__(CSR_THREADS)
void chunk_scatter_kernel(const uint32_t *chunk_list, const uint32_t *chunk_count, uint32_t n_chunks, uint32_t first, const uint64_t *list_start,
                          uint32_t *cursor, uint64_t *list_chunks, uint32_t nl) {
	__shared__ uint32_t lh[CSR_LDS_LISTS];
	const bool priv = nl <= (uint32_t)CSR_LDS_LISTS;
	const uint64_t base = (uint64_t)blockIdx.x * CSR_THREADS * CSR_ITEMS;
	uint32_t myl[CSR_ITEMS], myr[CSR_ITEMS];
	if (priv) { for (uint32_t i = threadIdx.x; i < nl; i += CSR_THREADS) lh[i] = 0; __syncthreads(); }
#pragma unroll
	for (int j = 0; j < CSR_ITEMS; j++) {
		const uint64_t c = base + (uint64_t)j * CSR_THREADS + threadIdx.x;
		myl[j] = c < n_chunks ? chunk_list[c] : NO_CHUNK;
		if (myl[j] != NO_CHUNK && priv) myr[j] = atomicAdd(&lh[myl[j]], 1u);
	}
	if (priv) {
		__syncthreads();
		for (uint32_t i = threadIdx.x; i < nl; i += CSR_THREADS) { const uint32_t n = lh[i]; lh[i] = n ? atomicAdd(&cursor[i], n) : 0u; }
		__syncthreads();
	}
#pragma unroll
	for (int j = 0; j < CSR_ITEMS; j++) {
		const uint32_t l = myl[j];
		if (l == NO_CHUNK) continue;
		const uint64_t c = base + (uint64_t)j * CSR_THREADS + threadIdx.x;
		const uint32_t pos = priv ? lh[l] + myr[j] : atomicAdd(&cursor[l], 1u);
		list_chunks[list_start[l] + pos] = ((uint64_t)chunk_count[c] << 32) | (c + first);
	}
}
#endif

#ifndef KMR_INSTANCE_TU
__global__ void pool_records_kernel(const uint32_t *chunk_list, const uint32_t *chunk_count, uint32_t n_chunks, unsigned long long *total, unsigned long long *nvalid) {
	unsigned long long s = 0, v = 0;
	for (uint64_t c = blockIdx.x * (uint64_t)blockDim.x + threadIdx.x; c < n_chunks; c += (uint64_t)gridDim.x * blockDim.x)
		if (chunk_list[c] != NO_CHUNK) { s += chunk_count[c]; v++; }
	s = wave_sum(s); v = wave_sum(v);
	if ((threadIdx.x & 63) == 0) { atomicAdd(total, s); atomicAdd(nvalid, v); }
}
#endif

static const int PROBE_SLOTS = 8192, PROBE_SPLIT = 16, PROBE_LISTS = 64;
template <int W, bool EXT>
__global__ __launch_bounds__(256)
void distinct_probe_kernel(PoolView pool, const uint64_t *list_start, const uint64_t *list_chunks, uint64_t n_lists, uint32_t kb, uint32_t rot,
                           int bits1, uint32_t n_probes, unsigned long long *tables , unsigned long long *out) {
	typedef typename PoolRec<W, EXT>::type Rec;
	const uint32_t p = blockIdx.x / PROBE_SPLIT, part = blockIdx.x % PROBE_SPLIT;
	const uint64_t l = (uint64_t)p * n_lists / n_probes;
	const uint64_t c0 = list_start[l], c1 = list_start[l + 1];
	unsigned long long *fp = tables + (size_t)p * PROBE_SLOTS;
	int sel = 0; while (sel < 40 - bits1 && (((c1 - c0) * CH) >> sel) > 2000) sel++;
	unsigned long long mine = 0, fresh = 0, again = 0;
	constexpr int UNR = 4;
	const uint64_t nw = (uint64_t)(blockDim.x >> 6) * PROBE_SPLIT;
	for (uint64_t cb = c0 + (uint64_t)part * (blockDim.x >> 6) + (threadIdx.x >> 6); cb < c1; cb += nw * UNR) {
		uint64_t d[UNR]; Rec r[UNR];
#pragma unroll
		for (int u = 0; u < UNR; u++) { const uint64_t ci = cb + (uint64_t)u * nw; d[u] = ci < c1 ? list_chunks[ci] : 0ull; }
#pragma unroll
		for (int u = 0; u < UNR; u++) {
			r[u].w = 0.0f;
			if ((uint32_t)(threadIdx.x & 63) < (uint32_t)(d[u] >> 32)) r[u] = ((const Rec *)(pool.base + (size_t)(uint32_t)d[u] * CH * sizeof(Rec)))[threadIdx.x & 63];
		}
#pragma unroll
		for (int u = 0; u < UNR; u++) {
			if (r[u].w == 0.0f) continue;
			const uint64_t g = part_order<W>(r[u].key, kb, rot);
			if (sel && ((g << bits1) >> (64 - sel)) != 0) continue;
			mine++;
			const unsigned long long f = (part_hash<W>(r[u].key) & ~3ull) | 1ull;
			uint32_t s = (uint32_t)(f >> 40) & (PROBE_SLOTS - 1);
			for (int probe = 0; probe < PROBE_SLOTS; probe++) {
				const unsigned long long old = atomicCAS(&fp[s], 0ull, f);
				if (old == 0ull) { fresh++; break; }
				if ((old & ~2ull) == f) { if (!(old & 2ull) && !(atomicOr(&fp[s], 2ull) & 2ull)) again++; break; }
				s = (s + 1) & (PROBE_SLOTS - 1);
			}
		}
	}
	mine = wave_sum(mine); fresh = wave_sum(fresh); again = wave_sum(again);
	if ((threadIdx.x & 63) == 0) { if (mine) atomicAdd(&out[0], mine); if (fresh) atomicAdd(&out[1], fresh); if (again) atomicAdd(&out[2], again); }
}

template <int W, bool EXT>
__global__ void verify_lists_kernel(PoolView pool, const uint64_t *list_start, const uint64_t *list_chunks, uint64_t n_lists, int bits, uint32_t kb, uint32_t rot,
                                    unsigned long long *total, unsigned long long *misfiled, unsigned long long *zero_w) {
	typedef typename PoolRec<W, EXT>::type Rec;
	unsigned long long n = 0, bad = 0, zw = 0;
	for (uint64_t l = blockIdx.x; l < n_lists; l += gridDim.x) {
		for (uint64_t ci = list_start[l] + (threadIdx.x >> 6); ci < list_start[l + 1]; ci += blockDim.x >> 6) {
			const uint64_t d = list_chunks[ci];
			if ((uint32_t)(threadIdx.x & 63) < (uint32_t)(d >> 32)) {
				const Rec r = ((const Rec *)(pool.base + (size_t)(uint32_t)d * CH * sizeof(Rec)))[threadIdx.x & 63];
				n++;
				if (bits && (part_order<W>(r.key, kb, rot) >> (64 - bits)) != l) bad++;
				if (r.w == 0.0f) zw++;
			}
		}
	}
	n = wave_sum(n); bad = wave_sum(bad); zw = wave_sum(zw);
	if ((threadIdx.x & 63) == 0) { atomicAdd(total, n); atomicAdd(misfiled, bad); atomicAdd(zero_w, zw); }
}

__device__ __forceinline__ void bucket_count_add(uint32_t *counts, uint64_t bucket, bool live) {
	const int lane = (int)(threadIdx.x & 63);
	bool done = !live;
	for (int round = 0; round < 6; round++) {
		const unsigned long long pending = __ballot(!done);
		if (!pending) break;
// ... 402 lines not shown
```

kmernator_amd/csrc/kmr_superkmer.hpp:

```cpp
#ifndef KMR_SUPERKMER_HPP_
#define KMR_SUPERKMER_HPP_

#include "kmr_partition.hpp"
#include "kmr_buckets.hpp"

namespace kmr {

#ifndef KMR_SK_MAX_N
#define KMR_SK_MAX_N 128
#endif
static const uint32_t SK_CHUNK_G = 64;
static const uint32_t SK_MAX_N = KMR_SK_MAX_N;
static const int SK_WAVES = 3;
static const int SK_WINDOW = 16;
static const int SK_RR = 3, SKL_RR = 4;

#ifdef KMR_DEBUG_HOOKS
#define SK_DBG(flags, bit) (((flags) & (bit)) != 0)
#else
#define SK_DBG(flags, bit) false
#endif
struct SkTrackRec { uint32_t raw, good; unsigned long long end_ordinal; };
static const uint32_t SK_TRACK_MAX = 512;
struct SkTrackView { const unsigned long long *bounds; uint32_t n; unsigned int *d_unique, *d_single; };
// ... 10 lines not shown
	struct SkTrackRec *track;
	const double *Pk;
};

struct SkBoundary { uint64_t read; uint32_t t, good; unsigned long long ordinal; };
template <int W>
__global__ __launch_bounds__(64)
void sk_track_boundary_kernel(ReadsView rv, DevParams p, SkBoundary *bd, uint32_t n_bd) {
	const uint32_t i = blockIdx.x * blockDim.x + threadIdx.x;
	if (i >= n_bd) return;
	const uint64_t r = bd[i].read, b0 = rv.offsets[r], L = rv.offsets[r + 1] - b0;
	const uint32_t k = p.k, target = bd[i].t;
	const uint8_t *bs = rv.bases + b0, *qs = rv.quals ? rv.quals + b0 : nullptr;
	const bool isRef = !qs || (L > 0 && qs[0] == 127);
	const bool filt = p.subsample > 1 || p.num_parts > 1 || p.world > 1;
	Roller<W> roll; roll.init(k);
	double w = 0.0;
	uint32_t raw = 0, good = 0, nN = 0;
	unsigned long long ord = rv.stream_base + b0 + L;
	for (uint64_t j = 0; j < L; j++) {
		const uint32_t code = base_code(bs[j]);
		nN += code >> 2;
		if (j >= k) nN -= base_code(bs[j - k]) >> 2;
		if (filt) roll.push(code & 3u);
		if (j + 1 < k) continue;
		const uint64_t x = j + 1 - k;
		if (isRef) w = 1.0;
		else if (x % 1024 == 0 || w == 0.0) { w = 1.0; for (uint32_t jj = 0; jj < k; jj++) w *= p.P[qs[x + jj]]; }
		else w *= p.P[qs[x + k - 1]] / p.P[qs[x - 1]];
		if (nN) w = 0.0;
		bool mine = true;
		if (filt) {
			const Key<W> kf = roll.getFwd(), kr = roll.getRc();
			const Key<W> canon = key_le<W>(kf, kr) ? kf : kr;
			const uint64_t hash = key_hash<W>(canon, p.kb);
			if (p.subsample > 1 && hash % p.subsample != 0) mine = false;
			if (p.world > 1 && distributed_thread_id(hash, p.world) != p.rank) mine = false;
			if (p.num_parts > 1 && distributed_thread_id(hash, p.num_parts) != p.part_idx) mine = false;
		}
		if (!mine) continue;
		raw++;
		if ((float)w > p.min_weight) good++;
		if (raw == target) { ord = rv.stream_base + b0 + x + 1; break; }
	}
	bd[i].good = good; bd[i].ordinal = ord;
}

static const uint32_t SK_EXT_X = 5u;
__host__ __device__ __forceinline__ uint32_t sk_base_granules(uint32_t n, uint32_t k) { return (n + k - 1 + 63) / 64; }
__host__ __device__ __forceinline__ uint32_t sk_ext_granules(uint32_t n) { return (n + 7) / 8; }
__host__ __device__ __forceinline__ uint32_t sk_rec_granules(uint32_t n, uint32_t k, bool uniform, bool ext) { return 1 + sk_base_granules(n, k) + (uniform ? 0u : (n + 3) / 4) + (ext ? sk_ext_granules(n) : 0u); }
__device__ __forceinline__ uint32_t sk_hdr_n(uint32_t y) { return (y >> 8) & 0xffu; }
__device__ __forceinline__ bool sk_hdr_uniform(uint32_t y) { return ((y >> 16) & 1u) != 0; }
__device__ __forceinline__ uint32_t sk_hdr_granules(uint32_t y) { return (y >> 17) & 0x7fu; }
__device__ __forceinline__ uint64_t sk_hdr_ordinal(uint32_t x, uint32_t y) { return (uint64_t)x | ((uint64_t)(y & 0xffu) << 32); }
__device__ __forceinline__ bool sk_hdr_is_ext(uint32_t y) { return ((y >> 30) & 1u) != 0; }
__device__ __forceinline__ uint32_t sk_hdr_ext_left(uint32_t y) { return (y >> 24) & 7u; }
__device__ __forceinline__ uint32_t sk_hdr_ext_right(uint32_t y) { return (y >> 27) & 7u; }
__device__ __forceinline__ uint32_t sk_hdr_ext(uint32_t left, uint32_t right) { return (left << 24) | (right << 27) | (1u << 30); }
__device__ __forceinline__ uint4 sk_make_header(unsigned long long ord, uint32_t n, bool uniform, uint32_t granules, uint32_t ext, uint32_t mhash, uint32_t wbits) {
	return make_uint4((uint32_t)ord, (uint32_t)(ord >> 32) | (n << 8) | ((uniform ? 1u : 0u) << 16) | (granules << 17) | ext, mhash, wbits);
}
__device__ __forceinline__ uint32_t sk_pend_make(uint32_t start, uint32_t n, bool uniform, uint32_t pos) { return (1u << 31) | (pos << 25) | ((uniform ? 1u : 0u) << 24) | (n << 16) | start; }
static const uint32_t SK_PEND_ADDRESS = 1u << 30;
__device__ __forceinline__ uint32_t sk_pend_start(uint32_t q) { return q & 0xffffu; }
__device__ __forceinline__ uint32_t sk_pend_n(uint32_t q) { return (q >> 16) & 0xffu; }
__device__ __forceinline__ bool sk_pend_uniform(uint32_t q) { return ((q >> 24) & 1u) != 0; }
__device__ __forceinline__ uint32_t sk_pend_pos(uint32_t q) { return (q >> 25) & 15u; }
__device__ __forceinline__ bool sk_pend_is_address(uint32_t q) { return ((q >> 30) & 1u) != 0; }
__device__ __forceinline__ bool sk_pend_live(uint32_t q) { return (q >> 31) != 0; }

#ifndef KMR_INSTANCE_TU
__global__ void sk_state_init_kernel(unsigned long long *state, uint64_t n) {
	for (uint64_t i = blockIdx.x * (uint64_t)blockDim.x + threadIdx.x; i < n; i += (uint64_t)gridDim.x * blockDim.x) state[i] = ((unsigned long long)NO_CHUNK << 32) | SK_CHUNK_G;
}
#endif
#ifndef KMR_INSTANCE_TU
__global__ void sk_close_kernel(const unsigned long long *state, uint64_t n, uint32_t *chunk_count, uint32_t cap) {
	for (uint64_t i = blockIdx.x * (uint64_t)blockDim.x + threadIdx.x; i < n; i += (uint64_t)gridDim.x * blockDim.x) {
		const unsigned long long s = state[i];
		const uint32_t c = (uint32_t)(s >> 32), f = (uint32_t)s;
		if (c != NO_CHUNK && c < cap) chunk_count[c] = f < SK_CHUNK_G ? f : SK_CHUNK_G;
	}
}
#endif

__device__ __forceinline__ void sk_wave_lds_order() { asm volatile("" ::: "memory"); __builtin_amdgcn_wave_barrier(); asm volatile("" ::: "memory"); }

__device__ __forceinline__ uint32_t sk_wave_scan_u32(uint32_t x) {
	x += (uint32_t)__builtin_amdgcn_update_dpp(0, (int)x, 0x111, 0xf, 0xf, true);
	x += (uint32_t)__builtin_amdgcn_update_dpp(0, (int)x, 0x112, 0xf, 0xf, true);
	x += (uint32_t)__builtin_amdgcn_update_dpp(0, (int)x, 0x114, 0xf, 0xf, true);
	x += (uint32_t)__builtin_amdgcn_update_dpp(0, (int)x, 0x118, 0xf, 0xf, true);
	x += (uint32_t)__builtin_amdgcn_update_dpp(0, (int)x, 0x142, 0xa, 0xf, false);
	x += (uint32_t)__builtin_amdgcn_update_dpp(0, (int)x, 0x143, 0xc, 0xf, false);
	return x;
}

struct SkSlab { uint32_t base[2]; uint32_t next; uint32_t hot_list; unsigned long long hot_state; };
static const uint32_t SK_NO_LIST = 0xffffffffu, SK_LIST_LOCKED = 0xfffffffeu;
static const int SK_HOT_AFTER = 3;
__device__ __forceinline__ uint32_t sk_alloc_chunk(SkSlab *slab, const PoolView &pool) {
	const uint32_t idx = atomicAdd(&slab->next, 1u);
	uint32_t c;
	if (idx < 128u) c = slab->base[idx >> 6] + (idx & 63u);
	else c = atomicAdd(pool.head, 1u);
	if (c >= pool.cap) { atomicOr(pool.err, (uint32_t)ERR_POOL_FULL); return NO_CHUNK; }
	return c;
}
__device__ __forceinline__ uint64_t sk_append_settle(unsigned long long *state, uint32_t list, uint32_t g, unsigned long long old, SkSlab *slab, const PoolView &pool, bool &waits) {
	const uint32_t c = (uint32_t)(old >> 32), f = (uint32_t)old;
	if (f + g <= SK_CHUNK_G) return (uint64_t)c * SK_CHUNK_G + f;
	if (f <= SK_CHUNK_G) {
		if (c != NO_CHUNK) pool.chunk_count[c] = f;
		const uint32_t c2 = sk_alloc_chunk(slab, pool);
		if (c2 == NO_CHUNK) { atomicExch(state + list, ((unsigned long long)NO_CHUNK << 32) | (SK_CHUNK_G + 1)); return ~0ull; }
		pool.chunk_list[c2] = list;
		atomicExch(state + list, ((unsigned long long)c2 << 32) | g);
		return (uint64_t)c2 * SK_CHUNK_G;
	}
	waits = true;
	return ~0ull;
}
__device__ __forceinline__ uint64_t sk_append_hot(SkSlab *slab, uint32_t list, uint32_t g, const PoolView &pool) {
	for (int spin = 0; spin < 4096; spin++) {
		const unsigned long long old = atomicAdd(&slab->hot_state, (unsigned long long)g);
		const uint32_t c = (uint32_t)(old >> 32), f = (uint32_t)old;
		if (f + g <= SK_CHUNK_G) return (uint64_t)c * SK_CHUNK_G + f;
		if (f <= SK_CHUNK_G) {
			pool.chunk_count[c] = f;
			const uint32_t c2 = sk_alloc_chunk(slab, pool);
			if (c2 == NO_CHUNK) return ~0ull;
			pool.chunk_list[c2] = list; pool.chunk_count[c2] = 0;
			atomicExch(&slab->hot_state, ((unsigned long long)c2 << 32) | g);
			return (uint64_t)c2 * SK_CHUNK_G;
		}
	}
	atomicOr(pool.err, (uint32_t)ERR_POOL_FULL);
	return ~0ull;
}
__device__ __forceinline__ uint64_t sk_append(unsigned long long *state, uint32_t list, uint32_t g, SkSlab *slab, const PoolView &pool) {
	unsigned long long *word = state + list;
	for (int spin = 0; spin < (1 << 22); spin++) {
		if (spin >= SK_HOT_AFTER) {
			uint32_t hl = slab->hot_list;
			if (hl == SK_NO_LIST && atomicCAS(&slab->hot_list, SK_NO_LIST, SK_LIST_LOCKED) == SK_NO_LIST) {
				const uint32_t c2 = sk_alloc_chunk(slab, pool);
				if (c2 == NO_CHUNK) { slab->hot_list = SK_NO_LIST; return ~0ull; }
				pool.chunk_list[c2] = list; pool.chunk_count[c2] = 0;
				slab->hot_state = ((unsigned long long)c2 << 32) | g;
				__builtin_amdgcn_fence(__ATOMIC_RELEASE, "workgroup");
				__hip_atomic_store(&slab->hot_list, list, __ATOMIC_RELEASE, __HIP_MEMORY_SCOPE_WORKGROUP);
				return (uint64_t)c2 * SK_CHUNK_G;
			}
			hl = __hip_atomic_load(&slab->hot_list, __ATOMIC_ACQUIRE, __HIP_MEMORY_SCOPE_WORKGROUP);
			if (hl == list) return sk_append_hot(slab, list, g, pool);
		}
		const unsigned long long old = atomicAdd(word, (unsigned long long)g);
		const uint32_t c = (uint32_t)(old >> 32), f = (uint32_t)old;
		if (f + g <= SK_CHUNK_G) return (uint64_t)c * SK_CHUNK_G + f;
		if (f <= SK_CHUNK_G) {
			if (c != NO_CHUNK) pool.chunk_count[c] = f;
			const uint32_t c2 = sk_alloc_chunk(slab, pool);
			if (c2 == NO_CHUNK) {
				atomicExch(word, ((unsigned long long)NO_CHUNK << 32) | (SK_CHUNK_G + 1));
				return ~0ull;
// ... 2069 lines not shown
```

Measured before the change: 58.44 billion.

## Speculate uniform-quality lean extraction and verify on a side stream

Merges the read-length max probe and a sampled quality AND/OR probe into one kernel, which removes a separate host round trip. When the sampled qualities look uniform, lean extraction starts right away while the full quality-range scan runs on a side stream. If the full scan disagrees, the state is restored from a snapshot and the general extraction is rerun. It also caches the L1 pool head at sync time so CSR building can skip a device readback. It folds the CSR histogram into a rank pass so the scatter no longer needs a cursor memset or atomics. The cost is extra snapshot/restore kernels, a second stream, and a redo path on misprediction.

```diff
diff --git a/kmernator_amd/csrc/kmr_api.hip b/kmernator_amd/csrc/kmr_api.hip
--- a/kmernator_amd/csrc/kmr_api.hip
+++ b/kmernator_amd/csrc/kmr_api.hip
@@ -135,6 +135,8 @@
 	uint32_t e = 0; DevStats s;
 	HIPCHK(h, hipMemcpy(&e, h->derr.get<uint32_t>(), sizeof(e), hipMemcpyDeviceToHost));
 	HIPCHK(h, hipMemcpy(&s, h->dstats.get<DevStats>(), sizeof(s), hipMemcpyDeviceToHost));
+	h->l1_head_seen = 0;
+	if (h->l1.head) HIPCHK(h, hipMemcpy(&h->l1_head_seen, h->l1.head.get<unsigned int>(), 4, hipMemcpyDeviceToHost));
 #ifdef KMR_DEBUG_HOOKS
 	if (h->superkmer_mode) { if (dbg()) fprintf(stderr, "sk_extract windows: %llu general, %llu fast\n", s.claimed, s.inserted); s.claimed = 0; s.inserted = 0; }
 #endif
@@ -178,19 +180,31 @@
 
 const size_t EXTRACT_SMEM = (size_t)WAVES_PER_BLOCK * 2 * TILE_BUF;
 
-int prepare_units(kmr_handle *h, ReadsView &rv, uint32_t span = (uint32_t)TILE_SPAN) {
+struct BatchProbe { unsigned int max_len = 0, q_and = 255, q_or = 0; };
+int probe_batch(kmr_handle *h, const ReadsView &rv, const uint8_t *quals, BatchProbe &bp) {
+	bp = BatchProbe();
+	if (rv.n_reads == 0) return 0;
+	int rc = h->umax.reserve(h, "umax", 16); if (rc) return rc;
+	HIPCHK(h, hipMemsetAsync(h->umax.get<unsigned int>(), 0, 16, h->stream));
+	hipLaunchKernelGGL(batch_probe_kernel, dim3(grid_for(rv.n_reads)), dim3(256), 0, h->stream, rv.offsets, rv.n_reads, quals, h->umax.get<unsigned int>());
+	HIPCHK(h, hipGetLastError());
+	unsigned int got[4] = {0, 0, 0, 0};
+	HIPCHK(h, hipMemcpyAsync(got, h->umax.get<unsigned int>(), 16, hipMemcpyDeviceToHost, h->stream));
+	HIPCHK(h, hipStreamSynchronize(h->stream));
+	bp.max_len = got[0]; bp.q_and = ~got[1] & 0xffu; bp.q_or = got[2];
+	return 0;
+}
+int prepare_units(kmr_handle *h, ReadsView &rv, uint32_t span = (uint32_t)TILE_SPAN, const BatchProbe *known = nullptr) {
 	rv.u_start = rv.u_end = rv.u_read = nullptr; rv.n_units = 0;
 	const uint64_t n = rv.n_reads;
 	if (n == 0) return 0;
-	int rc = h->umax.reserve(h, "umax", 4); if (rc) return rc;
-	HIPCHK(h, hipMemsetAsync(h->umax.get<unsigned int>(), 0, 4, h->stream));
-	rc = h->ucnt.reserve(h, "ucnt", 4 * (n + 1)); if (rc) return rc;
+	BatchProbe bp;
+	if (known) bp = *known;
+	else { const int prc = probe_batch(h, rv, nullptr, bp); if (prc) return prc; }
+	if (bp.max_len <= span) return 0;
+	int rc = h->ucnt.reserve(h, "ucnt", 4 * (n + 1)); if (rc) return rc;
 	hipLaunchKernelGGL(unit_count_kernel, dim3(grid_for(n)), dim3(256), 0, h->stream, rv.offsets, n, h->k, span, h->ucnt.get<uint32_t>(), h->umax.get<unsigned int>());
 	HIPCHK(h, hipGetLastError());
-	unsigned int mx = 0;
-	HIPCHK(h, hipMemcpyAsync(&mx, h->umax.get<unsigned int>(), 4, hipMemcpyDeviceToHost, h->stream));
-	HIPCHK(h, hipStreamSynchronize(h->stream));
-	if (mx <= span) return 0;
 	rc = h->ufirst.reserve(h, "ufirst", 8 * (n + 1)); if (rc) return rc;
 	rc = exclusive_scan(h, h->ucnt.get<uint32_t>(), n, h->ufirst.get<uint64_t>()); if (rc) return rc;
 	uint64_t U = 0;
@@ -731,21 +745,23 @@
 }
 int add_reads_partition(kmr_handle *h, const ReadsView &rv, uint64_t total_bases) { return with_w_ext(h, [&](auto W, auto EXT) { return add_reads_partition_t<W(), EXT()>(h, rv, total_bases); }); }
 
-int build_csr(kmr_handle *h, HostPool &p, uint64_t nl, uint32_t first, uint64_t **list_start, uint64_t **list_chunks, uint32_t *n_chunks_out) {
+int build_csr(kmr_handle *h, HostPool &p, uint64_t nl, uint32_t first, uint64_t **list_start, uint64_t **list_chunks, uint32_t *n_chunks_out, bool head_known = false) {
 	unsigned int used = 0;
-	HIPCHK(h, hipStreamSynchronize(h->stream));
-	HIPCHK(h, hipMemcpy(&used, p.head.get<unsigned int>(), 4, hipMemcpyDeviceToHost));
+	if (head_known && &p == &h->l1) used = h->l1_head_seen;
+	else {
+		HIPCHK(h, hipMemcpyAsync(&used, p.head.get<unsigned int>(), 4, hipMemcpyDeviceToHost, h->stream));
+		HIPCHK(h, hipStreamSynchronize(h->stream));
+	}
 	if (used > p.cap) used = p.cap;
 	used = used > first ? used - first : 0;
-	uint32_t *cnt;
+	uint32_t *cnt, *rank;
 	{ int arc = arena_get(h, &cnt, nl); if (arc) return arc; arc = arena_get(h, list_start, nl + 1); if (arc) return arc;
-	  arc = arena_get(h, list_chunks, std::max<unsigned>(used, 1)); if (arc) return arc; }
+	  arc = arena_get(h, list_chunks, std::max<unsigned>(used, 1)); if (arc) return arc; arc = arena_get(h, &rank, std::max<unsigned>(used, 1)); if (arc) return arc; }
 	HIPCHK(h, hipMemsetAsync(cnt, 0, 4 * nl, h->stream));
 	const unsigned csr_grid = (unsigned)(((uint64_t)used + CSR_THREADS * CSR_ITEMS - 1) / (CSR_THREADS * CSR_ITEMS));
-	if (used) hipLaunchKernelGGL(chunk_hist_kernel, dim3(csr_grid), dim3(CSR_THREADS), 0, h->stream, p.chunk_list.get<uint32_t>() + first, used, cnt, (uint32_t)nl);
-	int rc = exclusive_scan(h, cnt, nl, *list_start); if (rc) return rc;
-	HIPCHK(h, hipMemsetAsync(cnt, 0, 4 * nl, h->stream));
-	if (used) hipLaunchKernelGGL(chunk_scatter_kernel, dim3(csr_grid), dim3(CSR_THREADS), 0, h->stream, p.chunk_list.get<uint32_t>() + first, p.chunk_count.get<uint32_t>() + first, used, first, *list_start, cnt, *list_chunks, (uint32_t)nl);
+	if (used) hipLaunchKernelGGL(chunk_rank_kernel, dim3(csr_grid), dim3(CSR_THREADS), 0, h->stream, p.chunk_list.get<uint32_t>() + first, used, cnt, rank, (uint32_t)nl);
+	int rc = exclusive_scan_queue(h, cnt, nl, *list_start); if (rc) return rc;
+	if (used) hipLaunchKernelGGL(chunk_scatter_kernel, dim3(csr_grid), dim3(CSR_THREADS), 0, h->stream, p.chunk_list.get<uint32_t>() + first, p.chunk_count.get<uint32_t>() + first, rank, used, first, *list_start, *list_chunks);
 	HIPCHK(h, hipGetLastError());
 	*n_chunks_out = used;
 	if (dbg()) {
@@ -1215,8 +1231,8 @@
 template <int W, int WIN, bool PACKED = false> int launch_sk_extract_lean(kmr_handle *h, const ReadsView &rv, const SkParams &sp, float wK, const DevParams *override_params = nullptr, const SkPacked *packed = nullptr) {
 	return launch_sk_tiles(h, sk_extract_lean_kernel<W, WIN, PACKED>, "sk_extract_lean", W, WIN, SKL_WAVES, SKL_MIN_BLOCKS, SKL_EXTRACT_SMEM, rv, sp, override_params ? *override_params : dev_params(h), sp, pool_view(h, h->l1), wK, PACKED ? *packed : SkPacked{});
 }
-int sk_uniform_weight(kmr_handle *h, const ReadsView &rv, bool &lean, float &wK) {
-	lean = false; wK = 1.0f;
+int sk_uniform_weight(kmr_handle *h, const ReadsView &rv, const BatchProbe &bp, bool may_speculate, bool &lean, float &wK, int &unverified) {
+	lean = false; wK = 1.0f; unverified = -1;
 	if (h->tune.no_lean_extract) return 0;
 	if (!rv.quals && h->uniform_q_hint < 0) { lean = true; return 0; }
 	if (h->qual_mixed || rv.n_reads == 0) return 0;
@@ -1227,19 +1243,52 @@
 		lean = true; wK = (float)h->hPk[q0];
 		return 0;
 	}
-	{ int rc = h->qrange.reserve(h, "qrange", 8); if (rc) return rc; }
-	const unsigned int init[2] = {255u, 0u};
-	HIPCHK(h, hipMemcpyAsync(h->qrange.get<unsigned int>(), init, 8, hipMemcpyHostToDevice, h->stream));
-	hipLaunchKernelGGL(sk_qual_range_kernel, dim3(num_cus(h) * 8), dim3(256), 0, h->stream, rv.quals, rv.offsets, rv.n_reads, h->qrange.get<unsigned int>());
-	HIPCHK(h, hipGetLastError());
-	unsigned int got[2] = {0, 0};
-	HIPCHK(h, hipMemcpyAsync(got, h->qrange.get<unsigned int>(), 8, hipMemcpyDeviceToHost, h->stream));
-	HIPCHK(h, hipStreamSynchronize(h->stream));
+	unsigned int got[2] = {bp.q_and, bp.q_or};
+	const bool guess = got[0] == got[1];
+	if (guess && !may_speculate) {
+		{ int rc = h->qrange.reserve(h, "qrange", 8); if (rc) return rc; }
+		const unsigned int init[2] = {255u, 0u};
+		HIPCHK(h, hipMemcpyAsync(h->qrange.get<unsigned int>(), init, 8, hipMemcpyHostToDevice, h->stream));
+		hipLaunchKernelGGL(sk_qual_range_kernel, dim3(num_cus(h) * 8), dim3(256), 0, h->stream, rv.quals, rv.offsets, rv.n_reads, h->qrange.get<unsigned int>());
+		HIPCHK(h, hipGetLastError());
+		HIPCHK(h, hipMemcpyAsync(got, h->qrange.get<unsigned int>(), 8, hipMemcpyDeviceToHost, h->stream));
+		HIPCHK(h, hipStreamSynchronize(h->stream));
+	}
 	if (got[0] != got[1]) { h->qual_mixed = got[0] < got[1]; return 0; }
 	const unsigned int q0 = got[0];
-	if (q0 == 127) { lean = true; wK = 1.0f; return 0; }
-	if (!(h->hP[q0] > 0.0)) return 0;
-	lean = true; wK = (float)h->hPk[q0];
+	if (q0 == 127) { lean = true; wK = 1.0f; }
+	else if (!(h->hP[q0] > 0.0)) return 0;
+	else { lean = true; wK = (float)h->hPk[q0]; }
+	if (guess && may_speculate) unverified = (int)q0;
+	return 0;
+}
+int sk_verify_begin(kmr_handle *h, const ReadsView &rv) {
+	const uint64_t nl = sk_list_count(h->sk_bits);
+	if (!h->side_stream) { HIPCHK(h, hipStreamCreateWithFlags(&h->side_stream, hipStreamNonBlocking)); HIPCHK(h, hipEventCreateWithFlags(&h->side_fork, hipEventDisableTiming)); }
+	int rc = h->qrange.reserve(h, "qrange", 8); if (rc) return rc;
+	rc = h->sk_saved.reserve(h, "sk_saved", 8 * nl + sizeof(SkCallSmall)); if (rc) return rc;
+	hipLaunchKernelGGL(sk_call_state_kernel, dim3(grid_for(nl)), dim3(256), 0, h->stream, h->sk_state.get<unsigned long long>(), nl, h->l1.head.get<unsigned int>(), h->derr.get<uint32_t>(), h->dstats.get<DevStats>(),
+	                   h->sk_saved.get<unsigned long long>(), (SkCallSmall *)(h->sk_saved.get<unsigned long long>() + nl), h->qrange.get<unsigned int>(), 0);
+	HIPCHK(h, hipGetLastError());
+	HIPCHK(h, hipEventRecord(h->side_fork, h->stream));
+	HIPCHK(h, hipStreamWaitEvent(h->side_stream, h->side_fork, 0));
+	hipLaunchKernelGGL(sk_qual_range_kernel, dim3(num_cus(h) * 8), dim3(256), 0, h->side_stream, rv.quals, rv.offsets, rv.n_reads, h->qrange.get<unsigned int>());
+	HIPCHK(h, hipGetLastError());
+	return 0;
+}
+int sk_verify_end(kmr_handle *h, unsigned int q0, bool &confirmed) {
+	unsigned int got[2] = {0, 0};
+	HIPCHK(h, hipMemcpyAsync(got, h->qrange.get<unsigned int>(), 8, hipMemcpyDeviceToHost, h->side_stream));
+	HIPCHK(h, hipStreamSynchronize(h->side_stream));
+	confirmed = got[0] == q0 && got[1] == q0;
+	return 0;
+}
+int sk_call_rollback(kmr_handle *h) {
+	const uint64_t nl = sk_list_count(h->sk_bits);
+	HIPCHK(h, hipStreamSynchronize(h->stream));
+	hipLaunchKernelGGL(sk_call_state_kernel, dim3(grid_for(nl)), dim3(256), 0, h->stream, h->sk_state.get<unsigned long long>(), nl, h->l1.head.get<unsigned int>(), h->derr.get<uint32_t>(), h->dstats.get<DevStats>(),
+	                   h->sk_saved.get<unsigned long long>(), (SkCallSmall *)(h->sk_saved.get<unsigned long long>() + nl), h->qrange.get<unsigned int>(), 1);
+	HIPCHK(h, hipGetLastError());
 	return 0;
 }
 uint32_t sk_dbg_flags(const char *name) {
@@ -1254,15 +1303,16 @@
 	const uint64_t n = rvAll.n_reads;
 	const DevParams dp = dev_params(h);
 	const bool filt = dp.subsample > 1 || dp.num_parts > 1 || (dp.sub_wnb | dp.sub_snb) != 0 || (dp.world > 1 && !h->sk_exchange);
-	bool lean = false; float wK = 1.0f;
-	if (!filt && !h->ext && !sp_debug_extract(h)) { int rcq = sk_uniform_weight(h, rvAll, lean, wK); if (rcq) return rcq; }
+	const uint64_t avg = n ? std::max<uint64_t>(1, total_bases / n) : 1;
+	const uint64_t sub_bases = h->tune.sub_batch_bases ? h->tune.sub_batch_bases : (1ull << 31);
+	const uint64_t chunk = std::max<uint64_t>(64, (sub_bases / avg) & ~63ull);
+	bool lean = false; float wK = 1.0f; int unverified = -1;
+	const bool want_verdict = !filt && !h->ext && !sp_debug_extract(h);
+	BatchProbe bp;
+	{ int rcp = probe_batch(h, rvAll, want_verdict && h->uniform_q_hint < 0 && !h->qual_mixed && !h->tune.no_lean_extract ? rvAll.quals : nullptr, bp); if (rcp) return rcp; }
+	const bool may_speculate = h->tune.speculative_extract && !h->sk_exchange && h->cfg.world_size <= 1 && !h->cfg.size_tracker && !h->packed_direct && n <= chunk;
+	if (want_verdict) { int rcq = sk_uniform_weight(h, rvAll, bp, may_speculate, lean, wK, unverified); if (rcq) return rcq; }
 	if (h->packed_direct && (!lean || h->cfg.size_tracker)) return fail(h, KMR_ERR_STATE, "internal: a packed batch handed to an extraction that wants text");
-	if (rvAll.n_reads) {
-		uint32_t wb; memcpy(&wb, &wK, 4);
-		if (!lean) h->sk_uni_mixed = true;
-		else if (h->sk_uni_w == SK_UNI_NONE) h->sk_uni_w = wb;
-		else if (h->sk_uni_w != wb) h->sk_uni_mixed = true;
-	}
 	if (!h->sk_state) {
 		const uint64_t est = h->cfg.estimated_raw_kmers ? h->cfg.estimated_raw_kmers : std::max<uint64_t>(total_bases, h->call_bases_hint) * std::max<uint32_t>(1, h->cfg.world_size);
 		const uint64_t per_list = h->ext ? (W > 1 ? 400 : 600) : ((h->tune.target_list == 2048 && W > 1) ? 700 : h->tune.target_list * 3 / 4);
@@ -1283,9 +1333,6 @@
 		hipLaunchKernelGGL(sk_state_init_kernel, dim3(grid_for(nl0)), dim3(256), 0, h->stream, h->sk_state.get<unsigned long long>(), nl0);
 		HIPCHK(h, hipGetLastError());
 	}
-	const uint64_t avg = n ? std::max<uint64_t>(1, total_bases / n) : 1;
-	const uint64_t sub_bases = h->tune.sub_batch_bases ? h->tune.sub_batch_bases : (1ull << 31);
-	const uint64_t chunk = std::max<uint64_t>(64, (sub_bases / avg) & ~63ull);
 	if (h->cfg.size_tracker && n) {
 		h->trk_n = 0;
 		{ int rc = h->trk.reserve(h, "trk", n * sizeof(SkTrackRec)); if (rc) return rc; }
@@ -1294,7 +1341,7 @@
 	for (uint64_t r = 0; r < n; r += chunk) {
 		const uint64_t m = std::min(chunk, n - r);
 		ReadsView rv = reads_slice(rvAll, r, m);
-		int rc = prepare_units(h, rv, h->packed_direct ? SK_PACKED_SPAN : (uint32_t)TILE_SPAN); if (rc) return rc;
+		int rc = prepare_units(h, rv, h->packed_direct ? SK_PACKED_SPAN : (uint32_t)TILE_SPAN, n <= chunk ? &bp : nullptr); if (rc) return rc;
 		const uint64_t bases = m * avg + avg;
 		if (!h->l1.base && r == 0 && h->cfg.world_size <= 1 && !h->sk_exchange && (h->cfg.estimated_raw_kmers || h->call_bases_hint > total_bases)) {
 			const double job_bases = h->cfg.estimated_raw_kmers ? (double)h->cfg.estimated_raw_kmers * (double)avg / (double)(avg > h->k ? avg - h->k + 1 : 1) : (double)h->call_bases_hint;
@@ -1306,6 +1353,7 @@
 			}
 		}
 		rc = pool_reserve(h, h->l1, (h->ext ? 2 : 1) * bases / SK_CHUNK_G + ((h->l1.base && !h->sk_exchange) ? 0 : sk_list_count(h->sk_bits)) + (uint64_t)num_cus(h) * SK_EXTRACT_WAVES_PER_CU * 130 + 64, true); if (rc) return rc;
+		if (unverified >= 0) { rc = sk_verify_begin(h, rvAll); if (rc) return rc; }
 		TimeSpan tb(h, KMR_TIME_BUILD), te(h, KMR_TIME_EXTRACT);
 		SkParams sp = sk_params(h);
 		if (h->cfg.size_tracker) sp.track = h->trk.get<SkTrackRec>() + r;
@@ -1318,7 +1366,26 @@
 			return lean ? launch_sk_extract_lean<W, WIN()>(h, rv, sp, wK) : launch_sk_extract<W, WIN(), false>(h, rv, sp);
 		});
 		te.end(); tb.end();
-		if (rc) return rc;
+		if (rc) { if (unverified >= 0) hipStreamSynchronize(h->side_stream); return rc; }
+		if (unverified >= 0) {
+			bool confirmed = false;
+			rc = sk_verify_end(h, (unsigned int)unverified, confirmed); if (rc) return rc;
+			unverified = -1;
+			if (!confirmed) {
+				rc = sk_call_rollback(h); if (rc) return rc;
+				h->qual_mixed = true; lean = false; wK = 1.0f; h->extract_redo++;
+				TimeSpan tb2(h, KMR_TIME_BUILD), te2(h, KMR_TIME_EXTRACT);
+				rc = with_win<W>(h->sk_win, [&](auto WIN) { return launch_sk_extract<W, WIN(), false>(h, rv, sp); });
+				te2.end(); tb2.end();
+				if (rc) return rc;
+			}
+		}
+	}
+	if (rvAll.n_reads) {
+		uint32_t wb; memcpy(&wb, &wK, 4);
+		if (!lean) h->sk_uni_mixed = true;
+		else if (h->sk_uni_w == SK_UNI_NONE) h->sk_uni_w = wb;
+		else if (h->sk_uni_w != wb) h->sk_uni_mixed = true;
 	}
 	if (h->cfg.size_tracker && n) {
 		std::vector<SkTrackRec> recs(n);
@@ -1674,7 +1741,7 @@
 	}
 	p.refined = h->sk_state && h->sk_fine_shift > 0;
 	if (p.refined) { rc = sk_refine_lists(h, p.nl); if (rc) return rc; }
-	rc = build_csr(h, h->l1, p.nl, 0, &p.ls, &p.lc, &p.nch); if (rc) return rc;
+	rc = build_csr(h, h->l1, p.nl, 0, &p.ls, &p.lc, &p.nch, !p.refined); if (rc) return rc;
 	rc = count_entry_buffers(h, p, G, sk_entry_slack(h), G / (p.f.has_singletons ? 8 : 3), G / 3, h->sk_exchange && h->cfg.world_size > 1); if (rc) return rc;
 	rc = sk_count_uniform<W>(h, p.tracking, p.uni, p.f.uni_wbits); if (rc) return rc;
 	h->last_count_uniform = p.uni;
@@ -1724,7 +1791,7 @@
 	hipLaunchKernelGGL(sk_close_kernel, dim3(grid_for(nl)), dim3(256), 0, h->stream, h->sk_state.get<unsigned long long>(), nl, h->l1.chunk_count.get<uint32_t>(), h->l1.cap);
 	HIPCHK(h, hipGetLastError());
 	uint64_t *ls = nullptr, *lc = nullptr; uint32_t nch = 0;
-	rc = build_csr(h, h->l1, nl, 0, &ls, &lc, &nch); if (rc) return rc;
+	rc = build_csr(h, h->l1, nl, 0, &ls, &lc, &nch, true); if (rc) return rc;
 	const uint64_t G = h->stats.raw_good_kmers;
 	uint64_t want = (uint64_t)((double)G * ((double)hi / (double)nl) / (f.has_singletons ? 6.0 : 2.5)) + sk_entry_slack(h);
 	if (h->tune.early_entry_share >= 0) { want = (uint64_t)((double)G * h->tune.early_entry_share) + 16384; h->early.ue.reset(); }
@@ -1865,6 +1932,7 @@
 void kmr_destroy(kmr_handle *h) {
 	if (!h) return;
 	if (h->stream) hipStreamSynchronize(h->stream);
+	if (h->side_stream) { hipStreamSynchronize(h->side_stream); hipStreamDestroy(h->side_stream); hipEventDestroy(h->side_fork); h->side_stream = nullptr; }
 	for (int which = 0; which < KMR_TIME_GROUPS; which++) for (auto &pr : h->pending_events[which]) { hipEventDestroy(pr.first); hipEventDestroy(pr.second); }
 	release<HandleMem>(h);
 	free_partition_state(h);
@@ -1886,13 +1954,14 @@
 	if (!h) return KMR_ERR_INVALID_ARG;
 	hipSetDevice(h->device);
 	HIPCHK(h, hipStreamSynchronize(h->stream));
+	if (h->side_stream) HIPCHK(h, hipStreamSynchronize(h->side_stream));
 	clear_map(h->weak); clear_map(h->sing);
 	int rc = 0;
 	if (h->partition_mode) {
 		if (h->l1.head) HIPCHK(h, hipMemsetAsync(h->l1.head.get<unsigned int>(), 0, 4, h->stream));
 		h->l1.used_ub = 0;
 		h->inserted_records = 0;
-		h->qual_mixed = false;
+		h->qual_mixed = false; h->extract_redo = 0;
 		h->sk_uni_w = SK_UNI_NONE; h->sk_uni_mixed = false; h->peer_uni_w = SK_UNI_NONE; h->peer_uni_mixed = false; h->peers_declare = false;
 		h->xr_lo = 0; h->xr_hi = ~0ull; h->early.active = false;
 		if (h->d_uni) { const uint32_t init[2] = {SK_UNI_NONE, 0u}; HIPCHK(h, hipMemcpyAsync(h->d_uni.get<uint32_t>(), init, 8, hipMemcpyHostToDevice, h->stream)); HIPCHK(h, hipStreamSynchronize(h->stream)); }
@@ -1949,6 +2018,7 @@
 	else if (k == "stream_lookups") h->tune.no_stream_lookups = value == 0;
 	else if (k == "long_list_chunks") h->tune.long_list_chunks = value < 2 ? 2 : (uint64_t)value;
 	else if (k == "lean_extract") h->tune.no_lean_extract = value == 0;
+	else if (k == "speculative_extract") h->tune.speculative_extract = value != 0;
 	else if (k == "uniform_count") h->tune.no_uniform_count = value == 0;
 	else if (k == "packed_direct") h->tune.no_packed_direct = value == 0;
 	else if (k == "pow2_lists") h->tune.pow2_lists = value != 0;
@@ -1996,6 +2066,8 @@
 	else if (k == "saturated_keys") *value = (double)h->last_saturated_keys;
 	else if (k == "saturated_batches") *value = (double)h->last_saturated_batches;
 	else if (k == "count_attempts") *value = (double)h->last_count_attempts;
+	else if (k == "extract_redo") *value = (double)h->extract_redo;
+	else if (k == "qual_sample_bytes") *value = (double)QUAL_SAMPLE_BYTES;
 	else if (k == "device_blocks_live") *value = (double)g_blocks_live.load();
 	else if (k == "filter_score_ms") *value = h->last_score_ms;
 	else if (k == "select_ms") *value = h->last_select_ms;
diff --git a/kmernator_amd/csrc/kmr_host.hpp b/kmernator_amd/csrc/kmr_host.hpp
--- a/kmernator_amd/csrc/kmr_host.hpp
+++ b/kmernator_amd/csrc/kmr_host.hpp
@@ -108,6 +108,7 @@
 };
 struct BuildMem {
 	DevBuf sk_state;
+	DevBuf sk_saved;
 	HostPool l1;
 	DevBuf work_counter;
 	DevBuf l1_state; bool l1_state_dirty = false;
@@ -148,6 +149,7 @@
 	bool pow2_lists = false;
 	bool no_packed_direct = false;
 	bool no_uniform_count = false;
+	bool speculative_extract = true;
 	bool no_lean_extract = false;
 	bool exchange_fail_once = false;
 	uint64_t dump_piece_bytes = 0;
@@ -211,6 +213,9 @@
 	uint64_t last_saturated_keys = 0, last_saturated_batches = 0;
 	int last_count_attempts = 0;
 	bool qual_mixed = false;
+	uint64_t extract_redo = 0;
+	hipStream_t side_stream = nullptr; hipEvent_t side_fork = nullptr;
+	unsigned int l1_head_seen = 0;
 	uint32_t sk_fine_shift = 0;
 	uint32_t sk_min_override = 0;
 	uint64_t xo_segcap = 0; std::vector<uint64_t> xo_counts; const void *xo_batch = nullptr; uint64_t xo_first = 0;
diff --git a/kmernator_amd/csrc/kmr_kernels.hpp b/kmernator_amd/csrc/kmr_kernels.hpp
--- a/kmernator_amd/csrc/kmr_kernels.hpp
+++ b/kmernator_amd/csrc/kmr_kernels.hpp
@@ -78,6 +78,37 @@
 };
 
 static const uint32_t UNIT_KMERS = 9216;
+static const uint32_t QUAL_SAMPLE_BYTES = 1u << 16;
+#ifndef KMR_INSTANCE_TU
+__global__ __launch_bounds__(256)
+void batch_probe_kernel(const uint64_t *offsets, uint64_t n, const uint8_t *quals, unsigned int *out) {
+	const uint64_t tid = blockIdx.x * (uint64_t)blockDim.x + threadIdx.x, nthreads = (uint64_t)gridDim.x * blockDim.x;
+	unsigned int mx = 0;
+	for (uint64_t r = tid; r < n; r += nthreads) {
+		const uint64_t L = offsets[r + 1] - offsets[r];
+		mx = L > mx ? (unsigned int)(L > 0xffffffffull ? 0xffffffffu : L) : mx;
+	}
+#pragma unroll
+	for (int off = 32; off > 0; off >>= 1) { unsigned int o = __shfl_xor(mx, off, 64); mx = o > mx ? o : mx; }
+	if ((threadIdx.x & 63) == 0 && mx > __hip_atomic_load(out, __ATOMIC_RELAXED, __HIP_MEMORY_SCOPE_AGENT)) atomicMax(out, mx);
+	if (!quals) return;
+	const uint64_t b0 = offsets[0], b1 = offsets[n], len = b1 - b0, S = QUAL_SAMPLE_BYTES;
+	const bool whole = len <= 2 * S;
+	const uint64_t total = whole ? len : 2 * S;
+	if (tid - (tid & 63) >= total) return;
+	unsigned int inv = 0, any = 0;
+	for (uint64_t i = tid; i < total; i += nthreads) {
+		const unsigned int c = quals[(whole || i < S) ? b0 + i : b1 - 2 * S + i];
+		inv |= ~c & 0xffu; any |= c;
+	}
+#pragma unroll
+	for (int off = 32; off > 0; off >>= 1) { inv |= (unsigned int)__shfl_xor((int)inv, off, 64); any |= (unsigned int)__shfl_xor((int)any, off, 64); }
+	if ((threadIdx.x & 63) == 0) {
+		if (inv & ~__hip_atomic_load(out + 1, __ATOMIC_RELAXED, __HIP_MEMORY_SCOPE_AGENT)) atomicOr(out + 1, inv);
+		if (any & ~__hip_atomic_load(out + 2, __ATOMIC_RELAXED, __HIP_MEMORY_SCOPE_AGENT)) atomicOr(out + 2, any);
+	}
+}
+#endif
 #ifndef KMR_INSTANCE_TU
 __global__ void unit_count_kernel(const uint64_t *offsets, uint64_t n, uint32_t k, uint32_t span, uint32_t *counts, unsigned int *maxLen) {
 	unsigned int mx = 0;
diff --git a/kmernator_amd/csrc/kmr_partition.hpp b/kmernator_amd/csrc/kmr_partition.hpp
--- a/kmernator_amd/csrc/kmr_partition.hpp
+++ b/kmernator_amd/csrc/kmr_partition.hpp
@@ -531,48 +531,42 @@
 static const int CSR_THREADS = 256, CSR_ITEMS = 16;
 #ifndef KMR_INSTANCE_TU
 __global__ __launch_bounds__(CSR_THREADS)
-void chunk_hist_kernel(const uint32_t *chunk_list, uint32_t n_chunks, uint32_t *list_nchunks, uint32_t nl) {
+void chunk_rank_kernel(const uint32_t *chunk_list, uint32_t n_chunks, uint32_t *list_nchunks, uint32_t *rank, uint32_t nl) {
 	__shared__ uint32_t lh[CSR_LDS_LISTS];
 	const bool priv = nl <= (uint32_t)CSR_LDS_LISTS;
+	const uint64_t base = (uint64_t)blockIdx.x * CSR_THREADS * CSR_ITEMS;
+	uint32_t myl[CSR_ITEMS], myr[CSR_ITEMS];
 	if (priv) { for (uint32_t i = threadIdx.x; i < nl; i += CSR_THREADS) lh[i] = 0; __syncthreads(); }
+#pragma unroll
+	for (int j = 0; j < CSR_ITEMS; j++) {
+		const uint64_t c = base + (uint64_t)j * CSR_THREADS + threadIdx.x;
+		myl[j] = c < n_chunks ? chunk_list[c] : NO_CHUNK;
+		if (myl[j] == NO_CHUNK) continue;
+		if (priv) myr[j] = atomicAdd(&lh[myl[j]], 1u);
+		else rank[c] = atomicAdd(&list_nchunks[myl[j]], 1u);
+	}
+	if (!priv) return;
+	__syncthreads();
+	for (uint32_t i = threadIdx.x; i < nl; i += CSR_THREADS) { const uint32_t n = lh[i]; lh[i] = n ? atomicAdd(&list_nchunks[i], n) : 0u; }
+	__syncthreads();
+#pragma unroll
+	for (int j = 0; j < CSR_ITEMS; j++) {
+		if (myl[j] == NO_CHUNK) continue;
+		rank[base + (uint64_t)j * CSR_THREADS + threadIdx.x] = lh[myl[j]] + myr[j];
+	}
+}
+#endif
+#ifndef KMR_INSTANCE_TU
+__global__ __launch_bounds__(CSR_THREADS)
+void chunk_scatter_kernel(const uint32_t *chunk_list, const uint32_t *chunk_count, const uint32_t *rank, uint32_t n_chunks, uint32_t first, const uint64_t *list_start, uint64_t *list_chunks) {
 	const uint64_t base = (uint64_t)blockIdx.x * CSR_THREADS * CSR_ITEMS;
+#pragma unroll
 	for (int j = 0; j < CSR_ITEMS; j++) {
 		const uint64_t c = base + (uint64_t)j * CSR_THREADS + threadIdx.x;
 		if (c >= n_chunks) break;
 		const uint32_t l = chunk_list[c];
 		if (l == NO_CHUNK) continue;
-		if (priv) atomicAdd(&lh[l], 1u); else atomicAdd(&list_nchunks[l], 1u);
-	}
-	if (priv) { __syncthreads(); for (uint32_t i = threadIdx.x; i < nl; i += CSR_THREADS) if (lh[i]) atomicAdd(&list_nchunks[i], lh[i]); }
-}
-#endif
-#ifndef KMR_INSTANCE_TU
-__global__ __launch_bounds__(CSR_THREADS)
-void chunk_scatter_kernel(const uint32_t *chunk_list, const uint32_t *chunk_count, uint32_t n_chunks, uint32_t first, const uint64_t *list_start,
-                          uint32_t *cursor, uint64_t *list_chunks, uint32_t nl) {
-	__shared__ uint32_t lh[CSR_LDS_LISTS];
-	const bool priv = nl <= (uint32_t)CSR_LDS_LISTS;
-	const uint64_t base = (uint64_t)blockIdx.x * CSR_THREADS * CSR_ITEMS;
-	uint32_t myl[CSR_ITEMS], myr[CSR_ITEMS];
-	if (priv) { for (uint32_t i = threadIdx.x; i < nl; i += CSR_THREADS) lh[i] = 0; __syncthreads(); }
-#pragma unroll
-	for (int j = 0; j < CSR_ITEMS; j++) {
-		const uint64_t c = base + (uint64_t)j * CSR_THREADS + threadIdx.x;
-		myl[j] = c < n_chunks ? chunk_list[c] : NO_CHUNK;
-		if (myl[j] != NO_CHUNK && priv) myr[j] = atomicAdd(&lh[myl[j]], 1u);
-	}
-	if (priv) {
-		__syncthreads();
-		for (uint32_t i = threadIdx.x; i < nl; i += CSR_THREADS) { const uint32_t n = lh[i]; lh[i] = n ? atomicAdd(&cursor[i], n) : 0u; }
-		__syncthreads();
-	}
-#pragma unroll
-	for (int j = 0; j < CSR_ITEMS; j++) {
-		const uint32_t l = myl[j];
-		if (l == NO_CHUNK) continue;
-		const uint64_t c = base + (uint64_t)j * CSR_THREADS + threadIdx.x;
-		const uint32_t pos = priv ? lh[l] + myr[j] : atomicAdd(&cursor[l], 1u);
-		list_chunks[list_start[l] + pos] = ((uint64_t)chunk_count[c] << 32) | (c + first);
+		list_chunks[list_start[l] + rank[c]] = ((uint64_t)chunk_count[c] << 32) | (c + first);
 	}
 }
 #endif
diff --git a/kmernator_amd/csrc/kmr_superkmer.hpp b/kmernator_amd/csrc/kmr_superkmer.hpp
--- a/kmernator_amd/csrc/kmr_superkmer.hpp
+++ b/kmernator_amd/csrc/kmr_superkmer.hpp
@@ -116,6 +116,17 @@
 		const uint32_t c = (uint32_t)(s >> 32), f = (uint32_t)s;
 		if (c != NO_CHUNK && c < cap) chunk_count[c] = f < SK_CHUNK_G ? f : SK_CHUNK_G;
 	}
+}
+#endif
+
+struct SkCallSmall { unsigned int head; uint32_t err; DevStats stats; };
+#ifndef KMR_INSTANCE_TU
+__global__ void sk_call_state_kernel(unsigned long long *state, uint64_t n, unsigned int *head, uint32_t *err, DevStats *stats, unsigned long long *saved, SkCallSmall *small, unsigned int *qrange, int restore) {
+	const uint64_t tid = blockIdx.x * (uint64_t)blockDim.x + threadIdx.x;
+	for (uint64_t i = tid; i < n; i += (uint64_t)gridDim.x * blockDim.x) { if (restore) state[i] = saved[i]; else saved[i] = state[i]; }
+	if (tid != 0) return;
+	if (restore) { *head = small->head; *err = small->err; *stats = small->stats; }
+	else { small->head = *head; small->err = *err; small->stats = *stats; qrange[0] = 255u; qrange[1] = 0u; }
 }
 #endif
 
```

Result: no change. 58.84 billion, median of 6 (+0.7%).
